# ssufujia/SPCBPT-OptiX7

Hardware: AMD Instinct MI355X
Metric: Mpaths/sec (whole node), SPCBPT, 1920x1080 (higher is better)
Workload: dtype f32; 1 GPU; bedroom scene read from glTF (986132 triangles, SAH BVH of 246804 quantised 4-wide nodes, depth 16), 1920x1080, SPCBPT: 100000 light paths + 2073600 eye paths per subframe, CONNECTION_N=3, subspace tuple: trained, light pass geometry 100000 cores x 1 paths x 52 slots (lane); warmup_steps_run=32, frames_in_flight=32, frames_per_eye_launch=32, light_passes_ahead=32, light_passes_per_launch=32, sampler_builds_ahead=32, parallelism=1 GPU, rccl_ranks=0

## Files before the change

### include/spcbpt.h

```cpp
#ifndef SPCBPT_H
#define SPCBPT_H

#include <stddef.h>
#include <stdint.h>

#ifdef __cplusplus
extern "C" {
#endif

#define SPCBPT_NUM_SUBSPACE 1000
#define SPCBPT_NUM_SUBSPACE_LIGHTSOURCE 200
#define SPCBPT_CONNECTION_N 3
#define SPCBPT_MIN_RR_RATE 0.3f
#define SPCBPT_SCENE_EPSILON 1e-3f

typedef enum spcbpt_status {
    SPCBPT_OK = 0,
    SPCBPT_ERR_INVALID_ARG = -1,
    SPCBPT_ERR_NO_DEVICE = -2,
    SPCBPT_ERR_HIP = -3,
    SPCBPT_ERR_UNKNOWN_ALG = -4,
    SPCBPT_ERR_STATE = -5,
    SPCBPT_ERR_CAPACITY = -6,
    SPCBPT_ERR_IO = -7
// ... 206 lines not shown
    int64_t pixels;
    double mean, max;
} spcbpt_film_error_stats;
int spcbpt_film_error_struct_size(void);
int spcbpt_film_error(spcbpt_ctx* ctx, spcbpt_film_error_stats* out);
int spcbpt_film_error_host(const float* accum_rgba, const float* m2n, int64_t n_pixels, spcbpt_film_error_stats* out);

#define SPCBPT_DENOISE_SIGMA_V 4.0f
int spcbpt_denoise_variance(spcbpt_ctx* ctx, const spcbpt_denoise_params* params);
int spcbpt_denoise_variance_host(const float* accum_rgba, const float* m2n, const float* albedo_rgba, const float* normal_depth_rgba,
                                 const float eye[3], const float U[3], const float V[3], const float W[3],
                                 int width, int height, const spcbpt_denoise_params* params, float* out_rgba);

typedef struct spcbpt_reproject_params {
    float sigma_n, sigma_x, max_history;
} spcbpt_reproject_params;
#define SPCBPT_REPROJECT_SIGMA_N 0.5f
#define SPCBPT_REPROJECT_SIGMA_X_FRACTION 0.002f
#define SPCBPT_REPROJECT_MAX_HISTORY 32.0f
int spcbpt_reproject_params_struct_size(void);
int spcbpt_history_capture(spcbpt_ctx* ctx, uint32_t frames);
int spcbpt_history_reproject(spcbpt_ctx* ctx, const spcbpt_reproject_params* params);
int spcbpt_history_resolve(spcbpt_ctx* ctx, uint32_t frames);
int spcbpt_history_reset(spcbpt_ctx* ctx);
int spcbpt_read_history(spcbpt_ctx* ctx, float* resolved_rgba, uint8_t* resolved_rgba8, float* prior_rgba, float* history_rgbn);
int spcbpt_history_reproject_host(const float eye[3], const float U[3], const float V[3], const float W[3], const float* normal_depth_rgba,
                                  const float eye_h[3], const float U_h[3], const float V_h[3], const float W_h[3],
                                  const float* history_normal_depth_rgba, const float* history_rgbn, int width, int height,
                                  const spcbpt_reproject_params* params, float sigma_x_default_diag, float* prior_out);
int spcbpt_history_resolve_host(const float* prior_rgba, const float* accum_rgba, uint32_t frames, int64_t n_pixels, float* out_rgba);

int spcbpt_history_denoise(spcbpt_ctx* ctx, const spcbpt_denoise_params* params);
int spcbpt_read_history_variance(spcbpt_ctx* ctx, float* resolved_var, float* prior_var, float* history_var);
int spcbpt_history_reproject_var_host(const float eye[3], const float U[3], const float V[3], const float W[3], const float* normal_depth_rgba,
                                      const float eye_h[3], const float U_h[3], const float V_h[3], const float W_h[3],
                                      const float* history_normal_depth_rgba, const float* history_rgbn, const float* history_var,
                                      int width, int height, const spcbpt_reproject_params* params, float sigma_x_default_diag,
                                      float* prior_out, float* prior_var_out);
int spcbpt_history_resolve_var_host(const float* prior_rgba, const float* prior_var, const float* accum_rgba, const float* m2n, uint32_t frames,
                                    int64_t n_pixels, float* out_rgba, float* out_var);
int spcbpt_history_denoise_host(const float* resolved_rgba, const float* resolved_var, const float* albedo_rgba, const float* normal_depth_rgba,
                                const float eye[3], const float U[3], const float V[3], const float W[3],
                                int width, int height, const spcbpt_denoise_params* params, float* out_rgba);

int spcbpt_get_counters(spcbpt_ctx* ctx, spcbpt_counters* out);
int spcbpt_reset_counters(spcbpt_ctx* ctx);
int spcbpt_debug_phase_clocks(spcbpt_ctx* ctx, uint64_t out[19]);
const char* spcbpt_build_source_hash(void);
const char* spcbpt_build_arithmetic(void);
int spcbpt_abi_struct_sizes(int32_t* sizes, int capacity);
int spcbpt_debug_spill_arm(spcbpt_ctx* ctx);
int spcbpt_debug_spill_count(spcbpt_ctx* ctx, uint64_t* words_written, int* entries_per_thread);

enum { SPCBPT_SAMPLER_SUBSPACE = 0, SPCBPT_SAMPLER_UNIFORM = 1 };
int spcbpt_set_connection_sampler(spcbpt_ctx* ctx, int mode);

typedef struct spcbpt_unit_eye_vertex {
    float position[3], normal[3], flux[3], color[3], last_position[3], rmis3[3];
    float pdf, single_pdf, last_normal_projection;
    int32_t material_id, subspace_id, depth, last_zone_id;
} spcbpt_unit_eye_vertex;
enum spcbpt_unit_op { SPCBPT_UNIT_BSDF = 0, SPCBPT_UNIT_TREE = 1, SPCBPT_UNIT_STAGE1 = 2, SPCBPT_UNIT_BSEARCH = 3, SPCBPT_UNIT_STAGE2 = 4,
                      SPCBPT_UNIT_UNIFORM = 5, SPCBPT_UNIT_CONNECT = 6, SPCBPT_UNIT_EYE_STEP = 7, SPCBPT_UNIT_SKY_MISS = 8,
                      SPCBPT_UNIT_STAGE2_GUIDED = 9, SPCBPT_UNIT_SORTED = 10, SPCBPT_UNIT_ENV = 11, SPCBPT_UNIT_ENV_TABLE = 12,
                      SPCBPT_UNIT_TEX = 13 };
int spcbpt_debug_unit(spcbpt_ctx* ctx, int op, const uint32_t* in, int in_words, uint32_t* out, int out_words, int n,
                      const float* aux, int aux_floats);

int spcbpt_debug_trace_bench(spcbpt_ctx* ctx, const float* rays, int n, int mode, int any, int repeat, float* out_t, int32_t* out_tri,
                             float* out_uv, int32_t* out_visible, double* avg_ms, uint64_t stats[5]);
int spcbpt_enable_counters(spcbpt_ctx* ctx, int enabled);

int spcbpt_stream(spcbpt_ctx* ctx, void** stream);
int spcbpt_sync(spcbpt_ctx* ctx);
int spcbpt_sync_light(spcbpt_ctx* ctx);
int spcbpt_launch_deferred(spcbpt_ctx* ctx, const char* alg, uint32_t subframe_index, int row_begin, int row_end, int row_step);
int spcbpt_merge_deferred(spcbpt_ctx* ctx, int keep);
int spcbpt_sync_film(spcbpt_ctx* ctx);
int spcbpt_launch_eye_batch(spcbpt_ctx* ctx, int n_frames, const uint32_t* subframes, int row_begin, int row_end, int row_step);
int spcbpt_launch_light_batch(spcbpt_ctx* ctx, uint32_t first_frame, int n_frames);
int spcbpt_build_sampler_batch(spcbpt_ctx* ctx, int n_builds);
int spcbpt_debug_batch_scratch(spcbpt_ctx* ctx, int64_t* bytes, int* frames, int* fallbacks);
int spcbpt_debug_read_sampling_tables(spcbpt_ctx* ctx, uint32_t* guide2, int capacity2, uint16_t* guide1, float* gamma_q);

int spcbpt_set_light_ahead(spcbpt_ctx* ctx, int on);
int spcbpt_get_pipeline_state(spcbpt_ctx* ctx, int* light_ahead, int* pending_passes, int* sampler_intact, int* deferred_outstanding);
int spcbpt_reuse_sampler(spcbpt_ctx* ctx);
int spcbpt_lvc_import_wait(spcbpt_ctx* ctx);

int spcbpt_kernel_time(spcbpt_ctx* ctx, const char* name, double* avg_ms, int* launches);
int spcbpt_reset_kernel_time(spcbpt_ctx* ctx);
int spcbpt_enable_kernel_timing(spcbpt_ctx* ctx, int enabled);

int spcbpt_trace_closest(spcbpt_ctx* ctx, const float* rays, int n,
                         float* out_t, int32_t* out_tri, float* out_uv);
int spcbpt_trace_any(spcbpt_ctx* ctx, const float* rays, int n, int32_t* out_visible);

typedef struct spcbpt_pretrace_path {
    float contri[3];
    float sample_pdf;
    float fix_pdf;
    int32_t begin_ind;
    int32_t end_ind;
    int32_t choice_id;
    int32_t pixel_id[2];
    int32_t valid;
    int32_t pad;
} spcbpt_pretrace_path;

typedef struct spcbpt_pretrace_node {
    float a_position[3];
    float b_position[3];
    float a_dir[3];
    float b_dir[3];
    float a_normal[3];
    float b_normal[3];
    float peak_pdf;
    int32_t path_id;
    int32_t label_a;
    int32_t label_b;
    int32_t valid;
    int32_t light_source;
} spcbpt_pretrace_node;

int spcbpt_set_pretrace(spcbpt_ctx* ctx, int num_core, int padding);

int spcbpt_train_records_count(spcbpt_ctx* ctx, int* n_paths, int* n_nodes);
int spcbpt_train_records_read(spcbpt_ctx* ctx, spcbpt_pretrace_path* paths, int cap_paths,
                              spcbpt_pretrace_node* nodes, int cap_nodes);
int spcbpt_train_records_import(spcbpt_ctx* ctx, const spcbpt_pretrace_path* paths, int n_paths,
                                const spcbpt_pretrace_node* nodes, int n_nodes);
int spcbpt_train_records_clear(spcbpt_ctx* ctx);

int spcbpt_preprocess(spcbpt_ctx* ctx, int target_paths, int target_q_paths, int train);
int spcbpt_preprocess_stage(spcbpt_ctx* ctx, int stage, int arg);
int spcbpt_get_gamma(spcbpt_ctx* ctx, float* gamma);

int spcbpt_checkpoint_write(const char* dir, const spcbpt_tree_node* eye_tree, int n_eye,
                            const spcbpt_tree_node* light_tree, int n_light, const float* q, const float* gamma);
int spcbpt_checkpoint_read(const char* dir, spcbpt_tree_node* eye_tree, int* n_eye, int cap_eye,
                           spcbpt_tree_node* light_tree, int* n_light, int cap_light, float* q, float* gamma,
                           int have_current_gamma);
int spcbpt_gamma_to_cmf(const float* gamma, float* cmf_gamma);
int spcbpt_checkpoint_save(spcbpt_ctx* ctx, const char* dir);
int spcbpt_checkpoint_load(spcbpt_ctx* ctx, const char* dir);

int spcbpt_image_load(const char* path, int* width, int* height, uint8_t* rgba, size_t capacity_bytes);

typedef struct spcbpt_viewer spcbpt_viewer;
typedef struct spcbpt_viewer_state {
    float eye[3], lookat[3], up[3];
    float U[3], V[3], W[3];
    float fov_y, aspect;
    int32_t width, height;
    uint32_t subframe_index;
    int32_t alg_id;
    int32_t should_close, one_frame_render_only, camera_changed;
    float render_fps;
} spcbpt_viewer_state;
int spcbpt_viewer_create(spcbpt_ctx* ctx, const float eye[3], const float lookat[3], const float up[3], float fov_y,
                         int width, int height, spcbpt_viewer** out);
void spcbpt_viewer_destroy(spcbpt_viewer* v);
int spcbpt_viewer_mouse_button(spcbpt_viewer* v, int button, int action, double x, double y);
int spcbpt_viewer_cursor_pos(spcbpt_viewer* v, double x, double y);
int spcbpt_viewer_scroll(spcbpt_viewer* v, double xscroll, double yscroll);
int spcbpt_viewer_window_size(spcbpt_viewer* v, int width, int height);
// ... 36 lines not shown
```

### spcbpt-optix7_amd/api.py

```python
from __future__ import annotations

import ctypes as C
import os
from dataclasses import dataclass, field
from typing import List, Optional

import numpy as np

NUM_SUBSPACE = 1000
NUM_SUBSPACE_LIGHTSOURCE = 200
CONNECTION_N = 3
ENV_EYE_SEES_SKY = 1
ENV_PT_SKY_SHADOW_ALONG_DIR = 2

_HERE = os.path.dirname(os.path.abspath(__file__))
LIB_PATH = os.path.join(_HERE, "csrc", "libspcbpt_hip.so")
FAST_LIB_PATH = os.path.join(_HERE, "csrc", "libspcbpt_hip_fast.so")


class Material(C.Structure):
    _fields_ = [("base_color", C.c_float * 3), ("metallic", C.c_float), ("roughness", C.c_float),
                ("specular", C.c_float), ("specular_tint", C.c_float), ("subsurface", C.c_float),
                ("sheen", C.c_float), ("sheen_tint", C.c_float), ("clearcoat", C.c_float),
                ("clearcoat_gloss", C.c_float), ("albedo_tex", C.c_int32), ("brdf", C.c_int32)]
# ... 597 lines not shown
    return et[:ne.value].copy(), lt[:nl.value].copy(), q, g.reshape(NUM_SUBSPACE, NUM_SUBSPACE)


def gamma_to_cmf(gamma):
    lib = load_library()
    g = np.ascontiguousarray(gamma, dtype=np.float32).reshape(-1)
    out = np.zeros_like(g)
    lib.spcbpt_gamma_to_cmf(g.ctypes.data, out.ctypes.data)
    return out.reshape(NUM_SUBSPACE, NUM_SUBSPACE)


def load_library(path: str = LIB_PATH):
    global _lib
    if _lib is not None:
        return _lib
    if os.environ.get("SPCBPT_LIB"):
        path = os.environ["SPCBPT_LIB"]
    if not os.path.exists(path):
        raise SpcbptError(f"{path} not built: run `python -c 'import __graft_entry__ as g; g.build()'` (no CPU fallback exists)")
    try:
        import torch
    except ImportError:
        pass
    lib = C.CDLL(path, mode=C.RTLD_GLOBAL)
    try:
        lib.spcbpt_build_source_hash.restype = C.c_char_p
        built = lib.spcbpt_build_source_hash().decode()
    except AttributeError:
        built = "none"
    if path in (LIB_PATH, FAST_LIB_PATH) and built != source_hash() and not os.environ.get("SPCBPT_ALLOW_STALE_LIB"):
        raise SpcbptError(f"{path} was built from other sources (library {built}, tree {source_hash()}): run `make -C spcbpt-optix7_amd/csrc`")
    vp, i32, u32, f32p = C.c_void_p, C.c_int, C.c_uint32, C.POINTER(C.c_float)
    sig = {
        "spcbpt_create": [C.POINTER(SceneDesc), i32, C.POINTER(vp)],
        "spcbpt_create_lit": [C.POINTER(SceneDesc), C.POINTER(MeshLight), i32, i32, C.POINTER(vp)],
        "spcbpt_mesh_light_struct_size": [],
        "spcbpt_light_info": [vp, i32, C.POINTER(i32), C.POINTER(C.c_float), C.POINTER(i32), C.POINTER(i32), C.POINTER(i32)],
        "spcbpt_mesh_light_table": [vp, i32, vp, i32, i32, vp, vp, vp, vp, C.POINTER(C.c_double), C.POINTER(i32)],
        "spcbpt_scene_file_mesh_lights": [vp, C.POINTER(C.POINTER(MeshLight)), C.POINTER(i32)],
        "spcbpt_destroy": [vp],
        "spcbpt_set_camera": [vp, f32p, f32p, f32p, f32p],
        "spcbpt_set_camera_lookat": [vp, f32p, f32p, f32p, C.c_float, C.c_float],
        "spcbpt_resize": [vp, i32, i32],
        "spcbpt_set_subspace": [vp, vp, i32, vp, i32, vp, vp],
        "spcbpt_set_light_trace": [vp, C.POINTER(LightTraceParams)],
        "spcbpt_launch": [vp, C.c_char_p, u32, i32, i32, i32],
        "spcbpt_build_sampler": [vp],
        "spcbpt_build_sampler_batch": [vp, C.c_int],
        "spcbpt_launch_eye_batch": [vp, i32, C.POINTER(u32), i32, i32, i32],
        "spcbpt_launch_light_batch": [vp, u32, i32],
        "spcbpt_lvc_export": [vp, C.POINTER(vp), C.POINTER(vp), C.POINTER(i32)],
        "spcbpt_lvc_import": [vp, vp, i32, i32],
        "spcbpt_set_environment": [vp, vp, i32, i32, vp, C.c_float],
        "spcbpt_get_environment": [vp, C.POINTER(i32), C.POINTER(i32), f32p, C.POINTER(C.c_float), C.POINTER(i32)],
        "spcbpt_set_environment_mode": [vp, i32],
        "spcbpt_get_environment_mode": [vp, C.POINTER(i32)],
        "spcbpt_hdr_load": [C.c_char_p, C.POINTER(i32), C.POINTER(i32), vp, C.c_size_t],
        "spcbpt_lvc_set_capacity": [vp, i32],
        "spcbpt_lvc_get_capacity": [vp, C.POINTER(i32), C.POINTER(i32)],
        "spcbpt_lvc_read": [vp, vp, i32, C.POINTER(i32)],
        "spcbpt_sampler_read": [vp, vp, vp, vp, i32, C.POINTER(i32), C.POINTER(i32)],
        "spcbpt_read_accum": [vp, vp],
        "spcbpt_read_frame": [vp, vp],
        "spcbpt_accum_device_ptr": [vp, C.POINTER(vp)],
        "spcbpt_clear_accum": [vp],
        "spcbpt_get_counters": [vp, C.POINTER(Counters)],
        "spcbpt_reset_counters": [vp],
        "spcbpt_debug_phase_clocks": [vp, C.POINTER(C.c_uint64)],
        "spcbpt_set_connection_sampler": [vp, i32],
        "spcbpt_debug_unit": [vp, i32, vp, i32, vp, i32, i32, vp, i32],
        "spcbpt_debug_trace_bench": [vp, vp, i32, i32, i32, i32, vp, vp, vp, vp, vp, vp],
        "spcbpt_debug_spill_arm": [vp],
        "spcbpt_debug_spill_count": [vp, C.POINTER(C.c_uint64), C.POINTER(i32)],
        "spcbpt_enable_counters": [vp, i32],
        "spcbpt_stream": [vp, C.POINTER(vp)],
        "spcbpt_sync": [vp], "spcbpt_sync_film": [vp], "spcbpt_merge_deferred": [vp, i32], "spcbpt_launch_deferred": [vp, C.c_char_p, u32, i32, i32, i32],
        "spcbpt_sync_light": [vp],
        "spcbpt_set_light_ahead": [vp, i32],
        "spcbpt_get_pipeline_state": [vp, C.POINTER(i32), C.POINTER(i32), C.POINTER(i32), C.POINTER(i32)],
        "spcbpt_reuse_sampler": [vp],
        "spcbpt_read_film": [vp, vp, vp],
        "spcbpt_debug_batch_scratch": [vp, C.POINTER(C.c_int64), C.POINTER(i32), C.POINTER(i32)],
        "spcbpt_debug_read_sampling_tables": [vp, vp, i32, vp, vp],
        "spcbpt_lvc_import_wait": [vp],
        "spcbpt_kernel_time": [vp, C.c_char_p, C.POINTER(C.c_double), C.POINTER(i32)],
        "spcbpt_reset_kernel_time": [vp],
        "spcbpt_enable_kernel_timing": [vp, i32],
        "spcbpt_trace_closest": [vp, vp, i32, vp, vp, vp],
        "spcbpt_trace_any": [vp, vp, i32, vp],
        "spcbpt_camera_splat": [f32p, f32p, f32p, f32p, i32, i32, f32p, f32p, f32p, C.POINTER(i32), C.POINTER(i32), f32p],
        "spcbpt_launch_features": [vp, u32, i32, i32, i32],
        "spcbpt_read_features": [vp, vp, vp],
        "spcbpt_denoise": [vp, C.POINTER(DenoiseParams)],
        "spcbpt_denoise_params_struct_size": [],
        "spcbpt_read_denoised": [vp, vp, vp],
        "spcbpt_denoise_host": [f32p, f32p, f32p, f32p, f32p, f32p, f32p, i32, i32, C.POINTER(DenoiseParams), f32p],
        "spcbpt_set_film_moments": [vp, i32],
        "spcbpt_get_film_moments": [vp, C.POINTER(i32)],
        "spcbpt_read_film_moments": [vp, vp],
        "spcbpt_film_moments_update_host": [f32p, f32p, u32, C.c_int64, f32p],
        "spcbpt_film_error": [vp, C.POINTER(FilmErrorStats)],
        "spcbpt_film_error_struct_size": [],
        "spcbpt_film_error_host": [f32p, f32p, C.c_int64, C.POINTER(FilmErrorStats)],
        "spcbpt_denoise_variance": [vp, C.POINTER(DenoiseParams)],
        "spcbpt_history_capture": [vp, C.c_uint32], "spcbpt_history_reproject": [vp, C.POINTER(ReprojectParams)], "spcbpt_history_resolve": [vp, C.c_uint32],
        "spcbpt_history_reset": [vp], "spcbpt_reproject_params_struct_size": [], "spcbpt_read_history": [vp, vp, vp, vp, vp],
        "spcbpt_history_reproject_host": [f32p, f32p, f32p, f32p, f32p, f32p, f32p, f32p, f32p, f32p, f32p, i32, i32, C.POINTER(ReprojectParams), C.c_float, f32p],
        "spcbpt_history_resolve_host": [f32p, f32p, C.c_uint32, C.c_int64, f32p],
        "spcbpt_history_denoise": [vp, C.POINTER(DenoiseParams)], "spcbpt_read_history_variance": [vp, vp, vp, vp],
        "spcbpt_history_reproject_var_host": [f32p, f32p, f32p, f32p, f32p, f32p, f32p, f32p, f32p, f32p, f32p, f32p, i32, i32, C.POINTER(ReprojectParams), C.c_float, f32p, f32p],
        "spcbpt_history_resolve_var_host": [f32p, f32p, f32p, f32p, C.c_uint32, C.c_int64, f32p, f32p],
        "spcbpt_history_denoise_host": [f32p, f32p, f32p, f32p, f32p, f32p, f32p, f32p, i32, i32, C.POINTER(DenoiseParams), f32p],
        "spcbpt_viewer_set_denoise": [vp, i32], "spcbpt_viewer_get_denoise": [vp, C.POINTER(i32)],
        "spcbpt_viewer_set_reproject": [vp, i32], "spcbpt_viewer_get_reproject": [vp, C.POINTER(i32), C.POINTER(i32)],
        "spcbpt_denoise_variance_host": [f32p, f32p, f32p, f32p, f32p, f32p, f32p, f32p, i32, i32, C.POINTER(DenoiseParams), f32p],
        "spcbpt_preprocess": [vp, i32, i32, i32],
        "spcbpt_set_pretrace": [vp, i32, i32],
        "spcbpt_train_records_count": [vp, C.POINTER(i32), C.POINTER(i32)],
        "spcbpt_train_records_read": [vp, vp, i32, vp, i32],
        "spcbpt_train_records_import": [vp, vp, i32, vp, i32],
        "spcbpt_train_records_clear": [vp],
        "spcbpt_preprocess_stage": [vp, i32, i32],
        "spcbpt_get_gamma": [vp, vp],
        "spcbpt_checkpoint_write": [C.c_char_p, vp, i32, vp, i32, vp, vp],
        "spcbpt_checkpoint_read": [C.c_char_p, vp, C.POINTER(i32), i32, vp, C.POINTER(i32), i32, vp, vp, i32],
        "spcbpt_gamma_to_cmf": [vp, vp],
        "spcbpt_viewer_create": [vp, f32p, f32p, f32p, C.c_float, i32, i32, C.POINTER(vp)],
        "spcbpt_viewer_mouse_button": [vp, i32, i32, C.c_double, C.c_double],
        "spcbpt_viewer_cursor_pos": [vp, C.c_double, C.c_double],
        "spcbpt_viewer_scroll": [vp, C.c_double, C.c_double],
        "spcbpt_viewer_window_size": [vp, i32, i32],
        "spcbpt_viewer_iconify": [vp, i32],
        "spcbpt_viewer_key": [vp, i32, i32],
        "spcbpt_viewer_set_fps": [vp, C.c_float],
        "spcbpt_viewer_set_light_ahead": [vp, i32], "spcbpt_viewer_set_pipeline": [vp, i32],
        "spcbpt_viewer_frame": [vp],
        "spcbpt_viewer_get_state": [vp, C.POINTER(ViewerState)],
        "spcbpt_image_load": [C.c_char_p, C.POINTER(i32), C.POINTER(i32), vp, C.c_size_t],
        "spcbpt_checkpoint_save": [vp, C.c_char_p],
        "spcbpt_checkpoint_load": [vp, C.c_char_p],
        "spcbpt_gltf_load": [C.c_char_p, C.POINTER(vp), C.c_char_p, i32],
        "spcbpt_scene_file_load": [C.c_char_p, C.c_char_p, C.POINTER(vp)],
        "spcbpt_scene_file_desc": [vp, C.POINTER(SceneDesc)],
        "spcbpt_scene_file_camera": [vp, f32p, f32p, f32p, f32p, C.POINTER(i32), C.POINTER(i32)],
        "spcbpt_scene_file_environment": [vp, C.POINTER(vp), C.POINTER(i32), C.POINTER(i32), f32p, C.POINTER(C.c_float)],
        "spcbpt_scene_file_free": [vp],
        "spcbpt_get_subspace": [vp, vp, C.POINTER(i32), i32, vp, C.POINTER(i32), i32, vp, vp],
        "spcbpt_scene_info": [vp, C.POINTER(i32), C.POINTER(i32), C.POINTER(i32)],
    }
    for name, args in sig.items():
        if os.environ.get("SPCBPT_LIB") and not hasattr(lib, name):
            continue
        fn = getattr(lib, name)
        fn.argtypes = args
        fn.restype = C.c_int
    lib.spcbpt_viewer_destroy.argtypes = [vp]
    lib.spcbpt_viewer_destroy.restype = None
    lib.spcbpt_viewer_alg_name.argtypes = [i32]
    lib.spcbpt_viewer_alg_name.restype = C.c_char_p
    lib.spcbpt_last_error.argtypes = [vp]
    lib.spcbpt_last_error.restype = C.c_char_p
    lib.spcbpt_build_arithmetic.restype = C.c_char_p
    lib.spcbpt_scene_file_warnings.argtypes = [vp]
    lib.spcbpt_scene_file_warnings.restype = C.c_char_p
    _lib = lib
    return lib


EXPORTED_SYMBOLS = [
    "spcbpt_create", "spcbpt_create_lit", "spcbpt_mesh_light_struct_size", "spcbpt_light_info", "spcbpt_mesh_light_table", "spcbpt_scene_file_mesh_lights", "spcbpt_destroy", "spcbpt_last_error", "spcbpt_set_camera", "spcbpt_set_camera_lookat",
    "spcbpt_resize", "spcbpt_set_subspace", "spcbpt_set_light_trace", "spcbpt_launch", "spcbpt_launch_eye_batch", "spcbpt_launch_light_batch", "spcbpt_build_sampler", "spcbpt_build_sampler_batch",
    "spcbpt_lvc_export", "spcbpt_lvc_import", "spcbpt_lvc_set_capacity", "spcbpt_lvc_get_capacity", "spcbpt_set_environment", "spcbpt_get_environment", "spcbpt_set_environment_mode", "spcbpt_get_environment_mode", "spcbpt_hdr_load", "spcbpt_lvc_read", "spcbpt_sampler_read", "spcbpt_read_accum",
    "spcbpt_read_frame", "spcbpt_accum_device_ptr", "spcbpt_clear_accum", "spcbpt_get_counters",
    "spcbpt_reset_counters", "spcbpt_debug_phase_clocks", "spcbpt_debug_spill_arm", "spcbpt_debug_spill_count", "spcbpt_set_connection_sampler", "spcbpt_debug_unit", "spcbpt_debug_trace_bench",
    "spcbpt_build_source_hash", "spcbpt_build_arithmetic", "spcbpt_abi_struct_sizes", "spcbpt_lvc_export_on", "spcbpt_lvc_import_gathered", "spcbpt_lvc_export_batch_on", "spcbpt_lvc_import_gathered_batch", "spcbpt_film_pack_bands", "spcbpt_film_unpack_bands", "spcbpt_image_size", "spcbpt_get_light_trace", "spcbpt_enable_counters", "spcbpt_stream", "spcbpt_sync", "spcbpt_sync_light", "spcbpt_launch_deferred", "spcbpt_merge_deferred", "spcbpt_sync_film", "spcbpt_set_light_ahead", "spcbpt_get_pipeline_state", "spcbpt_reuse_sampler", "spcbpt_read_film", "spcbpt_debug_batch_scratch", "spcbpt_debug_read_sampling_tables", "spcbpt_lvc_import_wait", "spcbpt_kernel_time",
    "spcbpt_reset_kernel_time", "spcbpt_enable_kernel_timing", "spcbpt_trace_closest", "spcbpt_trace_any", "spcbpt_camera_splat",
    "spcbpt_launch_features", "spcbpt_read_features", "spcbpt_denoise", "spcbpt_denoise_params_struct_size", "spcbpt_read_denoised", "spcbpt_denoise_host",
    "spcbpt_set_film_moments", "spcbpt_get_film_moments", "spcbpt_read_film_moments", "spcbpt_film_moments_update_host", "spcbpt_film_error", "spcbpt_film_error_struct_size", "spcbpt_film_error_host", "spcbpt_denoise_variance", "spcbpt_denoise_variance_host",
    "spcbpt_history_capture", "spcbpt_history_reproject", "spcbpt_history_resolve", "spcbpt_history_reset", "spcbpt_read_history", "spcbpt_reproject_params_struct_size",
    "spcbpt_history_reproject_host", "spcbpt_history_resolve_host", "spcbpt_viewer_set_reproject", "spcbpt_viewer_get_reproject",
    "spcbpt_history_denoise", "spcbpt_read_history_variance", "spcbpt_history_reproject_var_host", "spcbpt_history_resolve_var_host", "spcbpt_history_denoise_host",
    "spcbpt_viewer_set_denoise", "spcbpt_viewer_get_denoise",
    "spcbpt_preprocess", "spcbpt_get_subspace", "spcbpt_scene_info", "spcbpt_set_pretrace", "spcbpt_train_records_count",
    "spcbpt_train_records_read", "spcbpt_train_records_import", "spcbpt_train_records_clear", "spcbpt_preprocess_stage",
    "spcbpt_get_gamma", "spcbpt_gltf_load", "spcbpt_scene_file_load", "spcbpt_scene_file_desc", "spcbpt_scene_file_camera",
    "spcbpt_scene_file_warnings", "spcbpt_scene_file_environment", "spcbpt_scene_file_free",
    "spcbpt_viewer_create", "spcbpt_viewer_destroy", "spcbpt_viewer_mouse_button", "spcbpt_viewer_cursor_pos", "spcbpt_viewer_scroll",
    "spcbpt_viewer_window_size", "spcbpt_viewer_iconify", "spcbpt_viewer_key", "spcbpt_viewer_set_fps", "spcbpt_viewer_set_light_ahead", "spcbpt_viewer_set_pipeline", "spcbpt_viewer_frame",
    "spcbpt_viewer_get_state", "spcbpt_viewer_alg_name",
    "spcbpt_image_load", "spcbpt_checkpoint_write", "spcbpt_checkpoint_read", "spcbpt_gamma_to_cmf", "spcbpt_checkpoint_save", "spcbpt_checkpoint_load",
]


def _fp(a):
    return a.ctypes.data_as(C.POINTER(C.c_float))


class Renderer:

    def __init__(self, scene: Scene, device: int = 0):
        self.lib = load_library()
        self.scene = scene
        sd, keep = scene.desc()
        h = C.c_void_p()
        if scene.mesh_lights:
            ml = scene.mesh_light_array()
            rc = self.lib.spcbpt_create_lit(C.byref(sd), ml, len(scene.mesh_lights), device, C.byref(h))
        else:
            rc = self.lib.spcbpt_create(C.byref(sd), device, C.byref(h))
        if rc != 0:
            msg = self.lib.spcbpt_last_error(None)
            raise SpcbptError(f"spcbpt_create failed ({rc}): {msg.decode() if msg else ''}")
        self.h = h
        self.width = self.height = 0
        self.lt = None

    def _chk(self, rc, what):
        if rc != 0:
            msg = self.lib.spcbpt_last_error(self.h)
            raise SpcbptError(f"{what} failed ({rc}): {msg.decode() if msg else ''}")

    def close(self):
        if getattr(self, "h", None):
            self.lib.spcbpt_destroy(self.h)
            self.h = None

    def __del__(self):
        try:
            self.close()
        except Exception:
            pass

    def set_camera(self, eye, U, V, W):
        a = [np.ascontiguousarray(x, dtype=np.float32) for x in (eye, U, V, W)]
        self._chk(self.lib.spcbpt_set_camera(self.h, *[_fp(x) for x in a]), "set_camera")

    def set_camera_lookat(self, eye, lookat, up, fov, aspect):
        a = [np.ascontiguousarray(x, dtype=np.float32) for x in (eye, lookat, up)]
        self._chk(self.lib.spcbpt_set_camera_lookat(self.h, *[_fp(x) for x in a], fov, aspect), "set_camera_lookat")

    def resize(self, w, h):
        self._chk(self.lib.spcbpt_resize(self.h, w, h), "resize")
        self.width, self.height = w, h

    def set_subspace(self, eye_tree=None, light_tree=None, q=None, cmf_gamma=None):
        if eye_tree is None and light_tree is None and q is None and cmf_gamma is None:
            self._chk(self.lib.spcbpt_set_subspace(self.h, None, 0, None, 0, None, None), "set_subspace")
            return
        et = np.ascontiguousarray(eye_tree, dtype=TREE_NODE_DTYPE)
        lt = np.ascontiguousarray(light_tree, dtype=TREE_NODE_DTYPE)
        q = np.ascontiguousarray(q, dtype=np.float32)
        g = np.ascontiguousarray(cmf_gamma, dtype=np.float32)
        assert q.size == NUM_SUBSPACE and g.size == NUM_SUBSPACE * NUM_SUBSPACE
        self._chk(self.lib.spcbpt_set_subspace(self.h, et.ctypes.data, et.shape[0], lt.ctypes.data, lt.shape[0],
                                               q.ctypes.data, g.ctypes.data), "set_subspace")

    def get_subspace(self, cap=1 << 20):
        et = np.zeros(cap, dtype=TREE_NODE_DTYPE)
# ... 126 lines not shown
        return out

    def read_features(self):
        self.image_size()
        a = np.zeros((self.height, self.width, 4), dtype=np.float32)
        n = np.zeros((self.height, self.width, 4), dtype=np.float32)
        self._chk(self.lib.spcbpt_read_features(self.h, a.ctypes.data, n.ctypes.data), "read_features")
        return a, n

    def read_film_moments(self):
        self.image_size()
        out = np.zeros((self.height, self.width, 4), dtype=np.float32)
        self._chk(self.lib.spcbpt_read_film_moments(self.h, out.ctypes.data), "read_film_moments")
        return out

    def history_capture(self, frames):
        self._chk(self.lib.spcbpt_history_capture(self.h, int(frames)), "history_capture")

    def history_reproject(self, sigma_n=0.0, sigma_x=0.0, max_history=0.0):
        p = ReprojectParams(float(sigma_n), float(sigma_x), float(max_history))
        self._chk(self.lib.spcbpt_history_reproject(self.h, C.byref(p)), "history_reproject")

    def history_resolve(self, frames):
        self._chk(self.lib.spcbpt_history_resolve(self.h, int(frames)), "history_resolve")

    def history_denoise(self, iterations=5, sigma_v=0.0, sigma_n=0.0, sigma_x=0.0):
        p = DenoiseParams(int(iterations), float(sigma_v), float(sigma_n), float(sigma_x))
        self._chk(self.lib.spcbpt_history_denoise(self.h, C.byref(p)), "history_denoise")

    def read_history_variance(self, resolved=True, prior=False, history=False):
        w, h = self.image_size()
        want = {"resolved": resolved, "prior": prior, "history": history}
        out = {k: np.zeros((h, w, 4), dtype=np.float32) for k, on in want.items() if on}
        self._chk(self.lib.spcbpt_read_history_variance(self.h, *[out[k].ctypes.data if k in out else None for k in want]), "read_history_variance")
        return out

    def history_reset(self):
        self._chk(self.lib.spcbpt_history_reset(self.h), "history_reset")

    def read_history(self, resolved=True, frame=True, prior=False, history=False):
        self.image_size()
        want = {"resolved": (resolved, np.float32), "frame": (frame, np.uint8), "prior": (prior, np.float32), "history": (history, np.float32)}
        out = {k: np.zeros((self.height, self.width, 4), dtype=t) for k, (on, t) in want.items() if on}
        self._chk(self.lib.spcbpt_read_history(self.h, *[out[k].ctypes.data if k in out else None for k in want]), "read_history")
        return out

    def read_denoised(self):
        self.image_size()
        d = np.zeros((self.height, self.width, 4), dtype=np.float32)
        f = np.zeros((self.height, self.width, 4), dtype=np.uint8)
        self._chk(self.lib.spcbpt_read_denoised(self.h, d.ctypes.data, f.ctypes.data), "read_denoised")
        return d, f

    def clear_accum(self):
        self._chk(self.lib.spcbpt_clear_accum(self.h), "clear_accum")

    def read_film(self, accum=True, frame=True):
        self.image_size()
        a = np.zeros((self.height, self.width, 4), dtype=np.float32) if accum else None
        f = np.zeros((self.height, self.width, 4), dtype=np.uint8) if frame else None
        self._chk(self.lib.spcbpt_read_film(self.h, a.ctypes.data if accum else None, f.ctypes.data if frame else None), "read_film")
        return a, f

    def pipeline_state(self):
        v = [C.c_int32() for _ in range(4)]
        self._chk(self.lib.spcbpt_get_pipeline_state(self.h, *[C.byref(x) for x in v]), "get_pipeline_state")
        return dict(zip(("light_ahead", "pending_passes", "sampler_intact", "deferred"), (int(x.value) for x in v)))

    def reuse_sampler(self):
        self._chk(self.lib.spcbpt_reuse_sampler(self.h), "reuse_sampler")

    def batch_scratch(self):
        b, f, k = C.c_int64(), C.c_int32(), C.c_int32()
        self._chk(self.lib.spcbpt_debug_batch_scratch(self.h, C.byref(b), C.byref(f), C.byref(k)), "debug_batch_scratch")
        return {"bytes": int(b.value), "frames": int(f.value), "fallbacks": int(k.value)}

    def sampling_tables(self, vertex_count):
        g2 = np.zeros(max(vertex_count, 1), dtype=np.uint32)
        g1 = np.zeros((NUM_SUBSPACE, 1024), dtype=np.uint16)
        gq = np.zeros((NUM_SUBSPACE, NUM_SUBSPACE), dtype=np.float32)
        self._chk(self.lib.spcbpt_debug_read_sampling_tables(self.h, g2.ctypes.data if vertex_count > 0 else None, len(g2), g1.ctypes.data, gq.ctypes.data),
                  "debug_read_sampling_tables")
        return g2[:vertex_count], g1, gq

    def lvc_read(self, capacity=None):
        if capacity is None:
            capacity = self.lt.num_core * self.lt.core_padding if self.lt else 1 << 22
        out = np.zeros(capacity, dtype=LIGHT_VERTEX_DTYPE)
        n = C.c_int()
        self._chk(self.lib.spcbpt_lvc_read(self.h, out.ctypes.data, capacity, C.byref(n)), "lvc_read")
        return out[:n.value].copy()

    def lvc_import(self, verts: np.ndarray):
        v = np.ascontiguousarray(verts, dtype=LIGHT_VERTEX_DTYPE)
        self._chk(self.lib.spcbpt_lvc_import(self.h, v.ctypes.data, v.shape[0], 0), "lvc_import")

    def lvc_import_device(self, d_ptr: int, count: int):
        self._chk(self.lib.spcbpt_lvc_import(self.h, C.c_void_p(d_ptr), count, 1), "lvc_import")

    def set_environment(self, rgba, center=None, radius=0.0):
        a = np.ascontiguousarray(rgba, dtype=np.float32)
        assert a.ndim == 3 and a.shape[2] == 4
        c3 = None if center is None else np.ascontiguousarray(center, dtype=np.float32)
        self._chk(self.lib.spcbpt_set_environment(self.h, a.ctypes.data, a.shape[1], a.shape[0], None if c3 is None else c3.ctypes.data, float(radius)), "set_environment")

    def environment(self):
        w, h, n = C.c_int(), C.c_int(), C.c_int()
        c3 = np.zeros(3, np.float32)
        r = C.c_float()
        self._chk(self.lib.spcbpt_get_environment(self.h, C.byref(w), C.byref(h), _fp(c3), C.byref(r), C.byref(n)), "get_environment")
        f = C.c_int()
        self._chk(self.lib.spcbpt_get_environment_mode(self.h, C.byref(f)), "get_environment_mode")
        return dict(width=w.value, height=h.value, center=c3, radius=r.value, n_lights=n.value, flags=f.value)

    def set_environment_mode(self, flags: int):
        self._chk(self.lib.spcbpt_set_environment_mode(self.h, int(flags)), "set_environment_mode")

    def lvc_set_capacity(self, vertices: int):
        self._chk(self.lib.spcbpt_lvc_set_capacity(self.h, int(vertices)), "lvc_set_capacity")

    def lvc_capacity(self):
        v, n = C.c_int(), C.c_int()
        self._chk(self.lib.spcbpt_lvc_get_capacity(self.h, C.byref(v), C.byref(n)), "lvc_get_capacity")
        return v.value, n.value

    def lvc_export(self):
        dv, dc, cap = C.c_void_p(), C.c_void_p(), C.c_int()
        self._chk(self.lib.spcbpt_lvc_export(self.h, C.byref(dv), C.byref(dc), C.byref(cap)), "lvc_export")
        return dv.value, dc.value, cap.value

    def sampler_read(self, capacity=None):
        if capacity is None:
            capacity = self.lt.num_core * self.lt.core_padding if self.lt else 1 << 22
        sub = np.zeros(NUM_SUBSPACE, dtype=SUBSPACE_DTYPE)
        cmfs = np.zeros(capacity, dtype=np.float32)
        jump = np.zeros(capacity, dtype=np.int32)
        vc, pc = C.c_int(), C.c_int()
        self._chk(self.lib.spcbpt_sampler_read(self.h, sub.ctypes.data, cmfs.ctypes.data, jump.ctypes.data, capacity,
                                               C.byref(vc), C.byref(pc)), "sampler_read")
        return sub, cmfs[:vc.value].copy(), jump[:vc.value].copy(), vc.value, pc.value

    def accum_device_ptr(self):
        p = C.c_void_p()
        self._chk(self.lib.spcbpt_accum_device_ptr(self.h, C.byref(p)), "accum_device_ptr")
        return p.value

    def set_light_ahead(self, on: bool):
        self._chk(self.lib.spcbpt_set_light_ahead(self.h, int(on)), "set_light_ahead")

    def lvc_import_wait(self):
        self._chk(self.lib.spcbpt_lvc_import_wait(self.h), "lvc_import_wait")

    def sync_light(self):
        self._chk(self.lib.spcbpt_sync_light(self.h), "sync_light")

    def stream(self):
        p = C.c_void_p()
        self._chk(self.lib.spcbpt_stream(self.h, C.byref(p)), "stream")
        return p.value or 0

    def counters(self):
        c = Counters()
        self._chk(self.lib.spcbpt_get_counters(self.h, C.byref(c)), "get_counters")
        return c.as_dict()

    def phase_clocks(self):
# ... 99 lines not shown
```

### spcbpt-optix7_amd/csrc/capi.hip

```cpp
#include "capi_common.h"
#include "mesh_light.h"

using namespace spc;

static thread_local std::string g_create_error;

static int create_context(const spcbpt_scene_desc* sc, const spcbpt_mesh_light* ml, int n_ml, int device, spcbpt_ctx** out) {
    if (!sc || !out) { g_create_error = "null argument"; return SPCBPT_ERR_INVALID_ARG; }
    *out = nullptr;
    if (!ml) {
        if (!sc->vertices || !sc->indices || !sc->tri_material || sc->n_vertices < 3 || sc->n_triangles < 1 || sc->n_materials < 1 ||
            !sc->materials || sc->n_lights < 1 || !sc->lights) {
            g_create_error = "scene needs vertices, indices, tri_material, >=1 material and >=1 quad light";
            return SPCBPT_ERR_INVALID_ARG;
        }
    } else {
        if (!sc->vertices || !sc->indices || !sc->tri_material || sc->n_vertices < 3 || sc->n_triangles < 1 || sc->n_materials < 1 ||
            !sc->materials || sc->n_lights < 0 || (sc->n_lights > 0 && !sc->lights) || n_ml < 0 || sc->n_lights + n_ml < 1) {
            g_create_error = "scene needs vertices, indices, tri_material, >=1 material and >=1 light (quad or mesh)";
            return SPCBPT_ERR_INVALID_ARG;
        }
    }
    int ndev = 0;
    if (hipGetDeviceCount(&ndev) != hipSuccess || ndev <= 0) { g_create_error = "no HIP device available (the MI355X path has no CPU fallback)"; return SPCBPT_ERR_NO_DEVICE; }
// ... 94 lines not shown
    for (int i = 0; i < sc->n_lights; i++) {
        const spcbpt_quad_light& s = sc->lights[i];
        DLight L;
        memset(&L, 0, sizeof(L));
        float cr[3] = {s.u[1] * s.v[2] - s.u[2] * s.v[1], s.u[2] * s.v[0] - s.u[0] * s.v[2], s.u[0] * s.v[1] - s.u[1] * s.v[0]};
        float len = sqrtf(cr[0] * cr[0] + cr[1] * cr[1] + cr[2] * cr[2]);
        if (!(len > 0)) { g_create_error = "degenerate quad light"; delete c; return SPCBPT_ERR_INVALID_ARG; }
        float inv = 1.0f / len;
        for (int k = 0; k < 3; k++) {
            L.corner[k] = s.position[k]; L.u[k] = s.position[k] + s.u[k]; L.v[k] = s.position[k] + s.v[k];
            L.emission[k] = s.emission[k]; L.normal[k] = cr[k] * inv;
        }
        L.area = len; L.div_level = s.div_level; L.ss_base = ss_base; L.id = (int)lights.size();
        ss_base += s.div_level * s.div_level;
        lights.push_back(L);
        DMaterial d;
        memset(&d, 0, sizeof(d));
        d.base_color[0] = d.base_color[1] = d.base_color[2] = 1.0f; d.metallic = 1.0f; d.roughness = 1.0f; d.specular = 0.5f;
        d.sheen_tint = 0.5f; d.clearcoat_gloss = 1.0f; d.light_id = i;
        mats.push_back(d);
        uint32_t base = (uint32_t)(V.size() / 3);
        float p3[3] = {L.u[0] + L.v[0] - L.corner[0], L.u[1] + L.v[1] - L.corner[1], L.u[2] + L.v[2] - L.corner[2]};
        V.insert(V.end(), L.corner, L.corner + 3); V.insert(V.end(), L.u, L.u + 3); V.insert(V.end(), L.v, L.v + 3); V.insert(V.end(), p3, p3 + 3);
        const float quv[8] = {0, 0, 1, 0, 0, 1, 1, 1};
        UV.insert(UV.end(), quv, quv + 8);
        const uint32_t qi[6] = {base, base + 1, base + 3, base, base + 3, base + 2};
        I.insert(I.end(), qi, qi + 6);
        TM.push_back((int)mats.size() - 1); TM.push_back((int)mats.size() - 1);
        EM.push_back(1); EM.push_back(1);
        c->h_light_tris.push_back(2);
    }
    for (int j = 0; j < n_ml; j++) {
        const MeshLightTable& T = ml_tables[(size_t)j];
        const int n = (int)T.tri.size();
        DLight L;
        memset(&L, 0, sizeof(L));
        L.area = (float)T.area; L.div_level = T.n_patches; L.ss_base = ss_base; L.id = (int)lights.size(); L.type = 2;
        for (int k = 0; k < 3; k++) L.emission[k] = ml[j].emission[k];
        ss_base += T.n_patches;
        DMaterial d;
        memset(&d, 0, sizeof(d));
        d.base_color[0] = d.base_color[1] = d.base_color[2] = 1.0f; d.metallic = 1.0f; d.roughness = 1.0f; d.specular = 0.5f;
        d.sheen_tint = 0.5f; d.clearcoat_gloss = 1.0f; d.light_id = L.id;
        mats.push_back(d);
        const int padded = (n + 7) / 8 * 8 + 8, buckets = mesh_light_guide_buckets(n);
        std::vector<uint32_t> guide;
        build_mesh_light_guide(T.cmf, buckets, guide);
        const size_t rec_off = c->h_etable.size() / 4, cmf_off = rec_off + (size_t)MESH_LIGHT_REC_QUADS * n, guide_off = cmf_off + (size_t)padded / 4;
        c->h_etable.resize((guide_off + (size_t)buckets / 4) * 4, 0.0f);
        const int32_t words[6] = {(int32_t)rec_off, (int32_t)cmf_off, (int32_t)guide_off, n, buckets, padded};
        memcpy(L.corner, words, 12); memcpy(L.u, words + 3, 12);
        for (int i = 0; i < n; i++) {
            const int t = ml_tris[(size_t)j][(size_t)T.tri[(size_t)i]];
            const uint32_t base = (uint32_t)(V.size() / 3);
            float P[3][3];
            for (int v = 0; v < 3; v++) {
                memcpy(P[v], sc->vertices + 3 * (size_t)sc->indices[3 * (size_t)t + v], 12);
                V.insert(V.end(), P[v], P[v] + 3);
                UV.push_back((float)T.patch[(size_t)i] + 0.5f); UV.push_back(0.0f);
                I[3 * (size_t)t + v] = base + (uint32_t)v;
            }
            TM[(size_t)t] = (int)mats.size() - 1;
            EM[(size_t)t] = 1;
            float* r = &c->h_etable[(rec_off + (size_t)MESH_LIGHT_REC_QUADS * i) * 4];
            for (int k = 0; k < 3; k++) { r[k] = P[0][k]; r[4 + k] = P[1][k] - P[0][k]; r[8 + k] = P[2][k] - P[0][k]; }
            r[3] = T.cmf[(size_t)i];
            memcpy(r + 7, &T.patch[(size_t)i], 4);
        }
        float* cm = &c->h_etable[cmf_off * 4];
        for (int i = 0; i < padded; i++) cm[i] = i < n ? T.cmf[(size_t)i] : 2.0f;
        memcpy(&c->h_etable[guide_off * 4], guide.data(), (size_t)buckets * 4);
        lights.push_back(L);
        c->h_light_tris.push_back(n);
    }
    HostMesh mesh;
    mesh.vertices = V.data(); mesh.texcoords = UV.data(); mesh.indices = I.data(); mesh.tri_material = TM.data(); mesh.tri_emitter = EM.data();
    mesh.n_vertices = (int)(V.size() / 3); mesh.n_triangles = (int)(I.size() / 3);
    Lbvh bvh;
    build_lbvh(mesh, bvh);
    c->n_triangles = mesh.n_triangles; c->n_nodes = (int)(bvh.nodes.size() / 16); c->bvh_depth = bvh.depth;
    c->n_lights = (int)lights.size(); c->n_mats = (int)mats.size();

    CREATE_TRY(c->d_nodes.reserve(bvh.nodes.size() + bvh.pairs.size()));
    CREATE_TRY(c->d_tris.reserve(bvh.tris.size()));
    if (getenv("SPCBPT_NO_TRI_PAIRS")) {
        for (size_t i = 0; i < bvh.pairs.size() / 16; i++) { uint32_t fl; memcpy(&fl, &bvh.pairs[i * 16 + 15], 4); fl &= 0x80000000u; memcpy(&bvh.pairs[i * 16 + 15], &fl, 4); }
        bvh.n_paired = 0;
    }
    CREATE_TRY(hipMemcpy(c->d_nodes + bvh.nodes.size(), bvh.pairs.data(), bvh.pairs.size() * 4, hipMemcpyHostToDevice));
    c->n_paired = bvh.n_paired;
    CREATE_TRY(c->d_tri_orig.reserve(bvh.tri_orig.size()));
    CREATE_TRY(c->d_mats.reserve(mats.size()));
    CREATE_TRY(hipMemcpy(c->d_nodes, bvh.nodes.data(), bvh.nodes.size() * 4, hipMemcpyHostToDevice));
    CREATE_TRY(hipMemcpy(c->d_tris, bvh.tris.data(), bvh.tris.size() * 4, hipMemcpyHostToDevice));
    CREATE_TRY(hipMemcpy(c->d_tri_orig, bvh.tri_orig.data(), bvh.tri_orig.size() * 4, hipMemcpyHostToDevice));
    CREATE_TRY(hipMemcpy(c->d_mats, mats.data(), mats.size() * sizeof(DMaterial), hipMemcpyHostToDevice));
    c->h_lights = lights;
    for (int k = 0; k < 3; k++) { c->bbox_lo[k] = 1e30f; c->bbox_hi[k] = -1e30f; }
    for (size_t i = 0; i < V.size(); i += 3)
        for (int k = 0; k < 3; k++) { c->bbox_lo[k] = std::min(c->bbox_lo[k], V[i + k]); c->bbox_hi[k] = std::max(c->bbox_hi[k], V[i + k]); }
    std::vector<DTexture> texs;
    for (int i = 0; i < sc->n_textures; i++) {
        const spcbpt_texture& t = sc->textures[i];
        if (!t.rgba || t.width < 1 || t.height < 1) { g_create_error = "bad texture"; delete c; return SPCBPT_ERR_INVALID_ARG; }
        uint32_t* d = nullptr;
        CREATE_TRY(dev_alloc(&d, (size_t)t.width * t.height));
        c->d_tex_data.push_back(d);
        CREATE_TRY(hipMemcpy(d, t.rgba, (size_t)t.width * t.height * 4, hipMemcpyHostToDevice));
        texs.push_back(DTexture{d, t.width, t.height});
    }
    CREATE_TRY(c->d_tex.reserve(texs.size()));
    if (!texs.empty()) CREATE_TRY(hipMemcpy(c->d_tex, texs.data(), texs.size() * sizeof(DTexture), hipMemcpyHostToDevice));
    CREATE_TRY(c->d_set_counts_all.reserve((size_t)2 * Context::kMaxSets + 2));
    CREATE_TRY(hipMemset(c->d_set_counts_all, 0, (2 * Context::kMaxSets + 2) * sizeof(int)));
    for (int s = 0; s < c->n_sets; s++) {
        CREATE_TRY(c->sets[s].subspace.reserve((size_t)SPCBPT_NUM_SUBSPACE));
        c->sets[s].counts = c->d_set_counts_all + 2 * s;
    }
    {
        hipDeviceProp_t prop;
        CREATE_TRY(hipGetDeviceProperties(&prop, device));
        c->num_cus = prop.multiProcessorCount;
    }
    CREATE_TRY(c->d_work_counter.reserve((size_t)Context::kMaxRender + 2));
    for (int lane = 0; lane < 2; lane++) c->lanes[lane].work_counter = c->d_work_counter + Context::kMaxRender + lane;
    CREATE_TRY(c->d_diag.reserve((size_t)4));
    CREATE_TRY(hipMemset(c->d_diag, 0, 4 * sizeof(uint32_t)));
    if (const char* e = getenv("SPCBPT_DEBUG_SPILL_ENTRIES")) c->spill_entries_debug = std::max(0, atoi(e));
    CREATE_TRY(c->d_counters.reserve((size_t)C_COUNT));
    CREATE_TRY(hipMemset(c->d_counters, 0, C_COUNT * sizeof(unsigned long long)));
    memset(&c->kp, 0, sizeof(c->kp));
    if (c->upload_lights()) { g_create_error = c->error; delete c; return SPCBPT_ERR_HIP; }
    c->kp.scene.nodes = c->d_nodes; c->kp.scene.tris = c->d_tris; c->kp.scene.tri_base = c->n_nodes; c->kp.scene.tri_orig = c->d_tri_orig; c->kp.scene.mats = c->d_mats;
    c->kp.scene.lights = c->d_lights; c->kp.scene.tex = c->d_tex; c->kp.scene.n_lights = c->n_lights; c->kp.scene.n_mats = c->n_mats;
    CREATE_TRY(c->d_nodes_q.reserve((size_t)c->n_nodes * 16));
    launch_repack_nodes_quad(c->d_nodes, c->d_nodes_q, c->n_nodes, c->stream);
    CREATE_TRY(hipGetLastError());
    CREATE_TRY(hipStreamSynchronize(c->stream));
    c->kp.scene.nodes_q = getenv("SPCBPT_NO_QUAD_TAIL") ? nullptr : c->d_nodes_q.p;
    c->kp.scene.fan_tail = getenv("SPCBPT_NO_FAN_TAIL") ? 0 : 1;
    c->kp.scene.general = 0;
    for (const DMaterial& m : mats) if (m.brdf) c->kp.scene.general = 1;
    if (n_ml > 0) c->kp.scene.general = 1;
    c->kp.sampler_counts = c->sets[0].counts;
    c->kp.diag = c->d_diag;
    c->kp.row_step = 1;
    CREATE_TRY(hipDeviceSynchronize());
#undef CREATE_TRY
    *out = c;
    return SPCBPT_OK;
}

extern "C" {

int spcbpt_create(const spcbpt_scene_desc* sc, int device, spcbpt_ctx** out) { return create_context(sc, nullptr, 0, device, out); }

int spcbpt_create_lit(const spcbpt_scene_desc* sc, const spcbpt_mesh_light* mesh_lights, int n_mesh_lights, int device, spcbpt_ctx** out) {
    if (n_mesh_lights < 0 || (n_mesh_lights > 0 && !mesh_lights)) { g_create_error = "create_lit: null mesh-light array"; if (out) *out = nullptr; return SPCBPT_ERR_INVALID_ARG; }
    static const spcbpt_mesh_light none = {0, {0, 0, 0}, 1};
    return create_context(sc, n_mesh_lights > 0 ? mesh_lights : &none, n_mesh_lights, device, out);
}
int spcbpt_mesh_light_struct_size(void) { return (int)sizeof(spcbpt_mesh_light); }

int spcbpt_light_info(spcbpt_ctx* c, int light, int32_t* type, float* area, int32_t* n_triangles, int32_t* first_subspace, int32_t* n_patches) {
    CTX_CHECK(c);
    if (light < 0 || light >= (int)c->h_lights.size()) { c->error = "light_info: light index out of range (" + std::to_string(c->h_lights.size()) + " lights)"; return SPCBPT_ERR_INVALID_ARG; }
    const DLight& L = c->h_lights[(size_t)light];
    const DEnv& E = c->kp.scene.env;
    if (type) *type = L.type;
    if (area) *area = L.type == 1 ? 0.0f : L.area;
    if (n_triangles) *n_triangles = light < (int)c->h_light_tris.size() ? c->h_light_tris[(size_t)light] : 0;
    if (first_subspace) *first_subspace = SPCBPT_NUM_SUBSPACE - 1 - (L.type == 1 ? 0 : L.ss_base);
    if (n_patches) *n_patches = L.type == 1 ? E.div_level * E.div_level : (L.type == 2 ? L.div_level : L.div_level * L.div_level);
    return SPCBPT_OK;
}

int spcbpt_destroy(spcbpt_ctx* c) {
    if (!c) return SPCBPT_ERR_INVALID_ARG;
    spc_viewers_forget_context(c);
    (void)hipSetDevice(c->device);
    (void)c->sync_all();
    delete c;
    return SPCBPT_OK;
}

const char* spcbpt_build_arithmetic(void) {
#if defined(SPCBPT_FAST_MATH_BUILD)
    return "approx";
#else
    return "ieee";
#endif
}

const char* spcbpt_last_error(const spcbpt_ctx* c) { return c ? c->error.c_str() : g_create_error.c_str(); }


int spcbpt_set_camera(spcbpt_ctx* c, const float eye[3], const float U[3], const float V[3], const float W[3]) {
    CTX_CHECK(c);
    if (!eye || !U || !V || !W) { c->error = "null camera vector"; return SPCBPT_ERR_INVALID_ARG; }
    memcpy(c->kp.eye, eye, 12); memcpy(c->kp.U, U, 12); memcpy(c->kp.V, V, 12); memcpy(c->kp.W, W, 12);
    c->have_camera = true;
    return SPCBPT_OK;
}

int spcbpt_set_camera_lookat(spcbpt_ctx* c, const float eye[3], const float lookat[3], const float up[3], float fov, float aspect) {
    CTX_CHECK(c);
    if (!eye || !lookat || !up) { c->error = "null camera vector"; return SPCBPT_ERR_INVALID_ARG; }
    auto cross = [](const float* a, const float* b, float* r) { r[0] = a[1] * b[2] - a[2] * b[1]; r[1] = a[2] * b[0] - a[0] * b[2]; r[2] = a[0] * b[1] - a[1] * b[0]; };
    auto norm = [](float* v) { float inv = 1.0f / sqrtf(v[0] * v[0] + v[1] * v[1] + v[2] * v[2]); v[0] *= inv; v[1] *= inv; v[2] *= inv; };
    float W[3] = {lookat[0] - eye[0], lookat[1] - eye[1], lookat[2] - eye[2]}, U[3], V[3];
    float wlen = sqrtf(W[0] * W[0] + W[1] * W[1] + W[2] * W[2]);
    cross(W, up, U); norm(U);
    cross(U, W, V); norm(V);
    float vlen = wlen * tanf(0.5f * fov * 3.14159265358979323846f / 180.0f);
    for (int k = 0; k < 3; k++) V[k] *= vlen;
    float ulen = vlen * aspect;
// ... 134 lines not shown
```

### spcbpt-optix7_amd/csrc/capi_debug.hip

```cpp
#include "capi_common.h"

using namespace spc;

extern "C" {

int spcbpt_get_light_trace(spcbpt_ctx* c, spcbpt_light_trace_params* out) {
    CTX_CHECK(c);
    if (!out) return SPCBPT_ERR_INVALID_ARG;
    *out = c->lt;
    if (out->core_count == 0) out->core_count = out->num_core - out->core_begin;
    return SPCBPT_OK;
}
int spcbpt_image_size(spcbpt_ctx* c, int* w, int* h) { CTX_CHECK(c); if (w) *w = (int)c->kp.width; if (h) *h = (int)c->kp.height; return SPCBPT_OK; }

int spcbpt_lvc_read(spcbpt_ctx* c, spcbpt_light_vertex* out, int capacity, int* count) {
    CTX_CHECK(c);
    if (!count) return SPCBPT_ERR_INVALID_ARG;
    if (!c->sets[c->lset].lvc) { c->error = "no LVC"; return SPCBPT_ERR_STATE; }
    int rc = c->fetch_counts();
    if (rc) return rc;
    *count = c->lvc_count;
    if (!out) return SPCBPT_OK;
    if (capacity < c->lvc_count) { c->error = "lvc_read: buffer too small"; return SPCBPT_ERR_CAPACITY; }
    HIP_TRY(c, hipMemcpy(out, c->sets[c->lset].lvc, (size_t)c->lvc_count * sizeof(LightVertex), hipMemcpyDeviceToHost));
    return SPCBPT_OK;
}

int spcbpt_sampler_read(spcbpt_ctx* c, spcbpt_subspace* sub, float* cmfs, int32_t* jump, int capacity, int* vc, int* pc) {
    CTX_CHECK(c);
    if (!c->have_sampler) { c->error = "no sampler built"; return SPCBPT_ERR_STATE; }
    if (!sub || !vc || !pc) return SPCBPT_ERR_INVALID_ARG;
    if (c->sync_all()) return SPCBPT_ERR_HIP;
    std::vector<DSubspace> h(SPCBPT_NUM_SUBSPACE);
    const CacheSet& S = c->sets[c->eset];
    HIP_TRY(c, hipMemcpy(h.data(), S.subspace, h.size() * sizeof(DSubspace), hipMemcpyDeviceToHost));
    for (int i = 0; i < SPCBPT_NUM_SUBSPACE; i++) {
        sub[i].jump_bias = h[i].jump_bias; sub[i].id = i; sub[i].size = h[i].size; sub[i].sum_pmf = h[i].sum_pmf; sub[i].q = 0;
    }
    int hc[2] = {0, 0};
    HIP_TRY(c, hipMemcpy(hc, S.counts, sizeof(hc), hipMemcpyDeviceToHost));
    *vc = hc[0]; *pc = hc[1];
    if (cmfs && jump) {
        if (capacity < hc[0]) { c->error = "sampler_read: buffer too small"; return SPCBPT_ERR_CAPACITY; }
        HIP_TRY(c, hipMemcpy(cmfs, S.cmfs, (size_t)hc[0] * 4, hipMemcpyDeviceToHost));
        HIP_TRY(c, hipMemcpy(jump, S.jump, (size_t)hc[0] * 4, hipMemcpyDeviceToHost));
    }
    return SPCBPT_OK;
}

int spcbpt_read_accum(spcbpt_ctx* c, float* out) {
    CTX_CHECK(c);
    if (!out || !c->d_accum) { c->error = "no accum buffer"; return SPCBPT_ERR_STATE; }
    if (c->sync_all()) return SPCBPT_ERR_HIP;
    if (int rc = c->check_diag()) return rc;
    HIP_TRY(c, hipMemcpy(out, c->d_accum, (size_t)c->kp.width * c->kp.height * 16, hipMemcpyDeviceToHost));
    return SPCBPT_OK;
}
int spcbpt_read_frame(spcbpt_ctx* c, uint8_t* out) {
    CTX_CHECK(c);
    if (!out || !c->d_frame) { c->error = "no frame buffer"; return SPCBPT_ERR_STATE; }
    if (c->sync_all()) return SPCBPT_ERR_HIP;
    if (int rc = c->check_diag()) return rc;
    HIP_TRY(c, hipMemcpy(out, c->d_frame, (size_t)c->kp.width * c->kp.height * 4, hipMemcpyDeviceToHost));
    return SPCBPT_OK;
}
int spcbpt_read_film(spcbpt_ctx* c, float* accum_out, uint8_t* frame_out) {
    CTX_CHECK(c);
    if (!c->d_accum || !c->d_frame) { c->error = "no film (spcbpt_resize first)"; return SPCBPT_ERR_STATE; }
    if (!c->cstream) HIP_TRY(c, hipStreamCreateWithFlags(&c->cstream, hipStreamNonBlocking));
    if (c->last_merge_k >= 0) HIP_TRY(c, c->ev_merge[c->last_merge_k].wait_on(c->cstream));
    const size_t px = (size_t)c->kp.width * c->kp.height;
    if (accum_out) HIP_TRY(c, hipMemcpyAsync(accum_out, c->d_accum, px * 16, hipMemcpyDeviceToHost, c->cstream));
    if (frame_out) HIP_TRY(c, hipMemcpyAsync(frame_out, c->d_frame, px * 4, hipMemcpyDeviceToHost, c->cstream));
    HIP_TRY(c, hipStreamSynchronize(c->cstream));
    return c->check_diag();
}
int spcbpt_debug_batch_scratch(spcbpt_ctx* c, int64_t* bytes, int* frames, int* fallbacks) {
    CTX_CHECK(c);
    if (bytes) *bytes = c->sbb_keys ? (int64_t)((size_t)c->sbb_frames * c->sbb_capacity * 16 + (size_t)c->sbb_frames * sampler_build_hist_ints() * sizeof(int)) : 0;
    if (frames) *frames = c->sbb_frames;
    if (fallbacks) *fallbacks = c->sbb_fallbacks;
    return SPCBPT_OK;
}
int spcbpt_debug_read_sampling_tables(spcbpt_ctx* c, uint32_t* guide2, int capacity2, uint16_t* guide1, float* gamma_q) {
    CTX_CHECK(c);
    if (c->sync_all()) return SPCBPT_ERR_HIP;
    if (guide2) {
        if (!c->have_sampler) { c->error = "no sampler built"; return SPCBPT_ERR_STATE; }
        int hc[2] = {0, 0};
        HIP_TRY(c, hipMemcpy(hc, c->sets[c->eset].counts, sizeof(hc), hipMemcpyDeviceToHost));
        if (capacity2 < hc[0]) { c->error = "debug_read_sampling_tables: buffer too small"; return SPCBPT_ERR_CAPACITY; }
        HIP_TRY(c, hipMemcpy(guide2, c->sets[c->eset].guide, (size_t)hc[0] * 4, hipMemcpyDeviceToHost));
    }
    if ((guide1 || gamma_q) && !c->d_guide1) { c->error = "no subspace tuple installed"; return SPCBPT_ERR_STATE; }
    if (guide1) HIP_TRY(c, hipMemcpy(guide1, c->d_guide1, (size_t)SPCBPT_NUM_SUBSPACE * CMF_GUIDE1 * sizeof(uint16_t), hipMemcpyDeviceToHost));
    if (gamma_q) HIP_TRY(c, hipMemcpy(gamma_q, c->d_gamma_q, (size_t)SPCBPT_NUM_SUBSPACE * SPCBPT_NUM_SUBSPACE * sizeof(float), hipMemcpyDeviceToHost));
    return SPCBPT_OK;
}
int spcbpt_accum_device_ptr(spcbpt_ctx* c, void** p) {
    CTX_CHECK(c);
    if (!p || !c->d_accum) return SPCBPT_ERR_STATE;
    *p = c->d_accum;
    return SPCBPT_OK;
}
int spcbpt_clear_accum(spcbpt_ctx* c) {
    CTX_CHECK(c);
    if (!c->d_accum) return SPCBPT_ERR_STATE;
    if (c->deferred.active) { c->error = "clear_accum: a deferred frame is outstanding (its merge would land in the cleared film): spcbpt_merge_deferred(ctx, keep) first"; return SPCBPT_ERR_STATE; }
    if (c->sync_all()) return SPCBPT_ERR_HIP;
    HIP_TRY(c, hipMemsetAsync(c->d_accum, 0, (size_t)c->kp.width * c->kp.height * 16, c->rstreams[0]));
    if (c->d_m2n) HIP_TRY(c, hipMemsetAsync(c->d_m2n, 0, (size_t)c->kp.width * c->kp.height * 16, c->rstreams[0]));
    HIP_TRY(c, hipStreamSynchronize(c->rstreams[0]));
    return SPCBPT_OK;
}

int spcbpt_get_counters(spcbpt_ctx* c, spcbpt_counters* o) {
    CTX_CHECK(c);
    if (!o) return SPCBPT_ERR_INVALID_ARG;
    unsigned long long h[C_COUNT];
    if (c->sync_all()) return SPCBPT_ERR_HIP;
    HIP_TRY(c, hipMemcpy(h, c->d_counters, sizeof(h), hipMemcpyDeviceToHost));
    o->closest_rays = h[C_CLOSEST]; o->shadow_rays = h[C_SHADOW]; o->node_visits = h[C_NODE]; o->tri_tests = h[C_TRI];
    o->surface_vertices = h[C_VERTEX]; o->textured_hits = h[C_TEX]; o->tree_nodes = h[C_TREE]; o->cmf_probes = h[C_CMF];
    o->connections = h[C_CONN]; o->gamma_q_reads = h[C_GQ]; o->lvc_stores = h[C_LVCW]; o->pixel_samples = h[C_PIX];
    o->eye_paths = h[C_EYE]; o->light_paths = h[C_LIGHT];
    return SPCBPT_OK;
}
int spcbpt_debug_phase_clocks(spcbpt_ctx* c, uint64_t out[19]) {
    CTX_CHECK(c);
    if (!out) return SPCBPT_ERR_INVALID_ARG;
    unsigned long long h[C_COUNT];
    if (c->sync_all()) return SPCBPT_ERR_HIP;
    HIP_TRY(c, hipMemcpy(h, c->d_counters, sizeof(h), hipMemcpyDeviceToHost));
    for (int i = 0; i < 5; i++) out[i] = h[C_PUBLIC + i] << 4;
    for (int i = 5; i < 9; i++) out[i] = h[C_PUBLIC + i];
    out[9] = h[C_T_SAMPLE] << 4;
    out[10] = h[C_W_START_MIN]; out[11] = h[C_W_END_MAX]; out[12] = h[C_W_END_SUM]; out[13] = h[C_W_WAVES]; out[14] = h[C_U_TAIL_SLOTS]; out[15] = h[C_U_TAIL_CLOSEST]; out[16] = h[C_U_TAIL_SHADOW]; out[17] = h[C_U_JOB_SLOTS]; out[18] = h[C_U_JOB_LANES];
    return SPCBPT_OK;
}
int spcbpt_reset_counters(spcbpt_ctx* c) {
    CTX_CHECK(c);
    if (c->sync_all()) return SPCBPT_ERR_HIP;
    HIP_TRY(c, hipMemsetAsync(c->d_counters, 0, C_COUNT * sizeof(unsigned long long), c->stream));
    HIP_TRY(c, hipMemsetAsync(c->d_counters + C_W_START_MIN, 0xff, sizeof(unsigned long long), c->stream));
    return SPCBPT_OK;
}
int spcbpt_enable_counters(spcbpt_ctx* c, int on) { CTX_CHECK(c); c->counting = on != 0; c->count_executed = on == 2; return SPCBPT_OK; }

int spcbpt_stream(spcbpt_ctx* c, void** s) { CTX_CHECK(c); if (!s) return SPCBPT_ERR_INVALID_ARG; *s = (void*)c->stream; return SPCBPT_OK; }
int spcbpt_set_light_ahead(spcbpt_ctx* c, int on) {
    CTX_CHECK(c);
    if (c->deferred.active) { c->error = "set_light_ahead: a deferred frame is outstanding: spcbpt_merge_deferred(ctx, keep) first"; return SPCBPT_ERR_STATE; }
    if (c->sync_all()) return SPCBPT_ERR_HIP;
    const bool was = c->light_ahead;
    c->light_ahead = on != 0;
    c->pending.clear();
    if (was && !c->light_ahead) { c->free_batch_build_scratch(); c->sbb_refused_bytes = 0; }
    return SPCBPT_OK;
}

int spcbpt_get_pipeline_state(spcbpt_ctx* c, int* light_ahead, int* pending_passes, int* sampler_intact, int* deferred_outstanding) {
    CTX_CHECK(c);
    if (light_ahead) *light_ahead = c->light_ahead ? 1 : 0;
    if (pending_passes) *pending_passes = (int)c->pending.size();
    if (sampler_intact) *sampler_intact = c->sampler_intact() ? 1 : 0;
    if (deferred_outstanding) *deferred_outstanding = c->deferred.active ? 1 : 0;
    return SPCBPT_OK;
}

int spcbpt_reuse_sampler(spcbpt_ctx* c) {
    CTX_CHECK(c);
    if (!c->sampler_intact()) { c->error = "reuse_sampler: the tables of the last sampler build are gone (a light pass, an import or a new tuple took their set)"; return SPCBPT_ERR_STATE; }
    c->have_sampler = true;
    return SPCBPT_OK;
}

int spcbpt_lvc_import_wait(spcbpt_ctx* c) {
    CTX_CHECK(c);
    if (c->import_gen >= 2 && c->ev_import[c->import_gen & 1]) HIP_TRY(c, hipEventSynchronize(c->ev_import[c->import_gen & 1]));
// ... 236 lines not shown
```

### spcbpt-optix7_amd/csrc/context.h

```cpp
#pragma once
#include <hip/hip_runtime.h>

#include <deque>
#include <map>
#include <string>
#include <type_traits>
#include <utility>
#include <vector>

#include "layout.h"
#include "reproject_pixel.h"

namespace spc {

struct Preprocessor;

struct TimedSpan {
    std::string name;
    hipEvent_t a, b;
    hipStream_t s;
};

template <class T>
static hipError_t dev_alloc(T** p, size_t n) {
// ... 42 lines not shown
struct CacheSet {
    DevBuf<LightVertex> lvc;
    DevBuf<LightVertex> lvc_sorted;
    DevBuf<uint32_t> jump;
    DevBuf<float> cmfs;
    DevBuf<uint32_t> guide;
    DevBuf<DSubspace> subspace;
    int* counts = nullptr;
    Event light;
    Event sampler, render;
    int render_event_of = 0;
    Event on_stream;
    int bound = -1;
    Event exch;
    int count_host = -1;
    bool light_counts_valid = false;
    int light_lane = 0;
};

struct LightLane {
    hipStream_t stream = nullptr;
    DevBuf<LightVertex> scratch;
    DevBuf<int> core_counts, core_offsets;
    DevBuf<uint32_t> keys, vals;
    DevBuf<float> weights;
    DevBuf<unsigned char> temp;
    DevBuf<uint32_t> spill;
    uint32_t* work_counter = nullptr;
};

struct Context {
    int device = 0;
    hipStream_t stream = nullptr;
    hipStream_t rstream = nullptr;
    hipStream_t cstream = nullptr;
    static const int kMaxRender = 8, kMaxSets = 128;
    int n_render = 2, n_sets = 6;
    hipStream_t rstreams[kMaxRender] = {};
    int rk = 0, last_merge_k = -1;
    DevBuf<float> d_result[kMaxRender];
    Event ev_merge[kMaxRender];
    CacheSet sets[kMaxSets];
    int lset = 0, eset = 0;
    std::deque<int> pending;
    bool light_ahead = false;
    int keys_set = -1;
    int export_on(hipStream_t xs, void** dv, void** dc, int* cap);
    int import_gathered(const void* shards, const int* counts_all, int world, int shard_cap, hipStream_t xs, int nf);
    int export_batch_on(hipStream_t xs, int nf, void* send, int* send_counts, int shard_cap);
    int wait_for_contents(hipStream_t xs, int s);
    hipEvent_t ev_import[2] = {};
    long long import_gen = 0;
    int* h_import_counts = nullptr;
    int* h_light_counts = nullptr;
    int build_set() const { return pending.empty() ? lset : pending.front(); }
    int begin_rewrite(hipStream_t ls, int s, int& waited_for);
    void set_rewritten(int s);
    int pass_traced(hipStream_t ls, int s, int lane);
    int sampler_built(int s);
    void contents_imported(int s, int count_host, int bound);
    template <class P>
    void sampler_tables(P& d, int s) const {
        const CacheSet& S = sets[s];
        d.lvc = S.lvc; d.lvc_sorted = S.lvc_sorted; d.subspace = S.subspace; d.cmfs = S.cmfs; d.guide = S.guide; d.sampler_counts = S.counts;
        if constexpr (std::is_same<P, KParams>::value) d.jump = reinterpret_cast<const int32_t*>(S.jump.p);
    }
    LightLane lanes[2];
    int light_toggle = 0;
    int ensure_lane_b();
    int light_pass_params(uint32_t frame, int n_frames, LightVertex* scratch, int* core_counts, bool count_events, DevBuf<uint32_t>& spill, int grid_cap);
    DevBuf<LightVertex> lb_scratch;
    DevBuf<int> lb_core_counts, lb_core_offsets, lb_path_counts;
    DevBuf<uint32_t> lb_spill;
    int launch_light_batch(uint32_t first_frame, int n);
    DevBuf<int> d_set_counts_all;
    DevBuf<uint32_t> d_spill_rs[kMaxRender];
    int sync_all();
    std::string error;
    KParams kp;
    DevBuf<float> d_nodes;
    DevBuf<float> d_nodes_q;
    DevBuf<float> d_nodes_q2;
    DevBuf<float> d_tris;
    int n_paired = 0;
    DevBuf<int32_t> d_tri_orig;
    DevBuf<DMaterial> d_mats;
    DLight* d_lights = nullptr;
    DevBuf<DTexture> d_tex;
    std::vector<uint32_t*> d_tex_data;
    int n_triangles = 0, n_nodes = 0, bvh_depth = 0, n_lights = 0, n_mats = 0;
    float* d_env_tex = nullptr;
    float* d_env_cmf = nullptr;
    std::vector<DLight> h_lights;
    std::vector<float> h_etable;
    std::vector<int> h_light_tris;
    int upload_lights();
    float bbox_lo[3] = {0, 0, 0}, bbox_hi[3] = {0, 0, 0};
    int set_environment(const float* rgba, int w, int h, const float* center, float radius);
    DevBuf<float> d_accum;
    DevBuf<uint32_t> d_frame;
    bool have_camera = false;
    float* d_eye_tree = nullptr;
    float* d_light_tree = nullptr;
    DevBuf<float> d_Q;
    DevBuf<float> d_gamma;
    DevBuf<float> d_gamma2;
    DevBuf<float> d_gamma_q;
    DevBuf<uint16_t> d_guide1;
    bool gamma_monotone = false;
    std::vector<spcbpt_tree_node> h_eye_tree, h_light_tree;
    std::vector<float> h_Q, h_gamma;
    bool have_subspace = false;
    bool tree_has_direction = false;
    spcbpt_light_trace_params lt = {100000, 52, 1, 0, 100000, 1};
    size_t lvc_capacity = 0;
    size_t lvc_fixed = 0;
    bool lvc_probe_needed = false;
    int probe_lvc_capacity();
    DevBuf<uint32_t> d_keys2;
    DevBuf<double> d_wsorted, d_prefix;
    DevBuf<int> d_hist;
    bool counting_build = true;
    int lvc_count = 0, path_count = 0;
    bool keys_ready = false, have_sampler = false;
    DevBuf<uint32_t> d_diag;
    int spill_entries_debug = -1;
    int spill_entries_needed() const;
    int check_diag();
    DevBuf<uint32_t> d_work_counter;
    int num_cus = 0, blocks_per_cu[3] = {0, 0, 0};
    int blocks_per_cu_batch = 0;
    int grid_percent = 0;
    int light_blocks_wide = -1;
    int light_blocks = -1;
    int light_batch_blocks = -1;
    int tiles_per_wave = 1;
    DevBuf<unsigned long long> d_counters;
    bool counting = false, timing = false;
    bool count_executed = false;
    int kernel_variant() const { return tree_has_direction ? 1 : (counting ? (count_executed ? 2 : 1) : 0); }
    std::vector<TimedSpan> spans;
    std::map<std::string, std::pair<double, int>> times;

    ~Context();
    void time_begin(const char* name, hipStream_t s = nullptr);
    void time_end();
    void resolve_spans();
    int ensure_spill(size_t threads, bool render = false);
    int ensure_temp(size_t bytes);
    int ensure_lvc_capacity(size_t n);
    int upload_tree(const spcbpt_tree_node* t, int n, float*& d_tree, std::vector<spcbpt_tree_node>& host_copy);
    int install_subspace(const spcbpt_tree_node* et, int ne, const spcbpt_tree_node* lt, int nl, const float* q, const float* g);
    int install_minimal_tuple();
    int set_light_trace(const spcbpt_light_trace_params& p);
    int launch_light(uint32_t frame);
    int fetch_counts();
    int fetch_counts_of(int set);
    int build_sampler();
    int build_sampler_batch(int n);
    DevBuf<uint32_t> sbb_keys; DevBuf<float> sbb_weights; DevBuf<double> sbb_wsorted; DevBuf<int> sbb_hist;
    int sbb_frames = 0; size_t sbb_capacity = 0;
    int sbb_fallbacks = 0;
    size_t sbb_refused_bytes = 0;
    void free_batch_build_scratch();
    size_t sbb_debug_limit() const;
    bool sampler_intact() const { return !built_sets.empty() && built_sets.back() == eset && sets[eset].sampler.set; }
    int launch_render(const char* name, bool spcbpt_alg, uint32_t frame, int r0, int r1, int rs, bool full_mis = false, bool defer_merge = false);
    struct Deferred { bool active = false; int rk = 0; uint32_t subframe = 0; int row_begin = 0, row_end = 0, row_step = 1; float* result = nullptr; } deferred;
    int merge_deferred(bool keep);
    int sync_film();
    std::deque<int> built_sets;
    int eye_batch = 1;
    DevBuf<float> d_result_b[kMaxRender][kMaxBatchFrames];
    DevBuf<FrameDesc> d_frames[kMaxRender];
    static const int kDescRing = 4;
    FrameDesc* h_frames = nullptr;
    hipEvent_t ev_desc[kMaxRender][kDescRing] = {};
    int desc_gen[kMaxRender] = {};
    int launch_eye_batch(int n, const uint32_t* subframes, int r0, int r1, int rs);
    DevBuf<float> d_splat[kMaxRender];
    int launch_splat(uint32_t frame, int r0, int r1, int rs);
    int film_ready();
    int begin_render(int r0, int r1, int rs);
    void next_render_stream();
    int chain_wait();
    int chain_end();
    int render_done(int s);
    int finish_frame();
    DevBuf<float> d_feat_albedo, d_feat_normal_depth;
    DevBuf<float> d_dn_position, d_dn_ping, d_dn_pong, d_denoised;
    DevBuf<uint32_t> d_denoised_frame;
    bool have_features = false, have_denoised = false;
    int launch_features(uint32_t subframe, int r0, int r1, int rs);
    int denoise(const spcbpt_denoise_params& p);
    void free_features();
    bool film_moments = false;
    DevBuf<float> d_m2n;
    DevBuf<unsigned char> d_err_scratch;
    int set_film_moments(bool on);
    int moments_step();
    int film_error(spcbpt_film_error_stats* out);
    int denoise_variance(const spcbpt_denoise_params& p);
    void free_moments();
    DevBuf<float> d_hist_rgbn, d_hist_normal_depth, d_prior, d_resolved;
    DevBuf<uint32_t> d_resolved_frame;
    ReprojectCamera hist_camera = {};
    uint32_t hist_width = 0, hist_height = 0;
    bool have_history = false, prior_live = false, have_resolved = false;
    int history_ready(const char* what, bool need_features);
    int resolve_into(uint32_t frames, float* out, uint32_t* frame, float* out_var = nullptr);
    int history_capture(uint32_t frames);
    int history_reproject(const spcbpt_reproject_params& p);
    int history_resolve(uint32_t frames);
    void free_history();
    DevBuf<float> d_hist_var, d_prior_var, d_resolved_var;
    bool have_hist_var = false, have_prior_var = false, have_resolved_var = false;
    bool history_variance_now() const;
    int history_denoise(const spcbpt_denoise_params& p);
    Preprocessor* pre = nullptr;
    spcbpt_pretrace_path* d_pre_paths = nullptr;
    spcbpt_pretrace_node* d_pre_nodes = nullptr;
    size_t pre_capacity = 0;
    int pre_num_core = 100000, pre_padding = 10, pre_last_added = 0;
    int set_pretrace(int num_core, int padding);
    int launch_pretrace(uint32_t iteration);
    int preprocess_stage(int stage, int arg);
    int preprocess(int target_paths, int target_q_paths, bool train);
    void free_preprocess();
};

}
```

### spcbpt-optix7_amd/csrc/ctx_state.hip

```cpp
#include "capi_common.h"

using namespace spc;

namespace spc {

void Context::time_begin(const char* name, hipStream_t s) {
    if (!timing) return;
    TimedSpan sp;
    sp.name = name;
    sp.s = s ? s : stream;
    (void)hipEventCreate(&sp.a);
    (void)hipEventCreate(&sp.b);
    (void)hipEventRecord(sp.a, sp.s);
    spans.push_back(sp);
}
void Context::time_end() {
    if (!timing || spans.empty()) return;
    (void)hipEventRecord(spans.back().b, spans.back().s);
}
int Context::sync_all() {
    HIP_TRY(this, hipStreamSynchronize(stream));
    if (lanes[1].stream) HIP_TRY(this, hipStreamSynchronize(lanes[1].stream));
    for (int k = 0; k < n_render; k++)
        if (rstreams[k] && rstreams[k] != stream) HIP_TRY(this, hipStreamSynchronize(rstreams[k]));
    return 0;
}
void Context::resolve_spans() {
    for (auto& sp : spans) {
        (void)hipEventSynchronize(sp.b);
        float ms = 0.f;
        if (hipEventElapsedTime(&ms, sp.a, sp.b) == hipSuccess) {
            auto& acc = times[sp.name];
            acc.first += ms;
            acc.second += 1;
        }
        (void)hipEventDestroy(sp.a);
        (void)hipEventDestroy(sp.b);
    }
    spans.clear();
}

int Context::spill_entries_needed() const {
    const int entries = std::max(0, 3 * bvh_depth - kStackLds);
    return spill_entries_debug >= 0 ? std::min(entries, spill_entries_debug) : entries;
}
int Context::check_diag() {
    if (!d_diag) return 0;
    uint32_t h[4] = {0, 0, 0, 0};
    HIP_TRY(this, hipMemcpy(h, d_diag, sizeof(h), hipMemcpyDeviceToHost));
    if (h[0] == 0 && h[1] == 0 && h[2] == 0) return 0;
    HIP_TRY(this, hipMemsetAsync(d_diag, 0, sizeof(h), stream));
    HIP_TRY(this, hipStreamSynchronize(stream));
    if (h[0] == 0 && h[1] == 0) {
        error = "light-vertex cache overflow: a light pass produced more vertices than a buffer set holds (" + std::to_string(lvc_capacity) +
                ", sized from a probe pass); frames since the last sync are invalid -- fix the capacity with spcbpt_lvc_set_capacity";
        return SPCBPT_ERR_CAPACITY;
    }
    if (h[0] == 0) {
        error = "LVC exchange: a rank's shard did not fit the agreed shard capacity (or the gathered cache did not fit the LVC); frames since the last sync are invalid -- raise the capacity (spcbpt_comm_set_shard_capacity)";
        return SPCBPT_ERR_CAPACITY;
    }
    error = "traversal stack overflow: " + std::to_string(h[0]) + " entries did not fit LDS + spill area (BVH depth " + std::to_string(bvh_depth) +
            ", spill entries per thread " + std::to_string(spill_entries_needed()) + "); results since the last sync are invalid";
    return SPCBPT_ERR_STATE;
}

int Context::ensure_spill(size_t threads, bool render) {
    const int entries = spill_entries_needed();
    kp.spill_entries = entries;
    if (entries == 0) { kp.spill = nullptr; return 0; }
    DevBuf<uint32_t>& buf = render ? d_spill_rs[rk] : lanes[0].spill;
    HIP_TRY(this, buf.reserve(threads * (size_t)entries));
    kp.spill = buf;
    return 0;
}

int Context::upload_tree(const spcbpt_tree_node* t, int n, float*& d_tree, std::vector<spcbpt_tree_node>& host_copy) {
    for (int i = 0; i < n; i++) {
        if (t[i].leaf) {
            if (t[i].label < 0 || t[i].label >= SPCBPT_NUM_SUBSPACE) { error = "tree label out of range"; return SPCBPT_ERR_INVALID_ARG; }
        } else {
            if (t[i].type < 0 || t[i].type > 2) { error = "tree node type out of range"; return SPCBPT_ERR_INVALID_ARG; }
            for (int k = 0; k < 8; k++)
                if (t[i].child[k] < 0 || t[i].child[k] >= n) { error = "tree child index out of range"; return SPCBPT_ERR_INVALID_ARG; }
        }
    }
    host_copy.assign(t, t + n);
    const size_t budget = (size_t)16 * n + 64;
    std::vector<float> packed(4);
    std::vector<int> src(1, 0);
    for (size_t slot = 0; slot < src.size(); slot++) {
        const spcbpt_tree_node& nd = t[src[slot]];
        uint32_t meta;
        if (nd.leaf) {
            meta = TREE_LEAF_BIT | (uint32_t)nd.label;
        } else {
            const size_t base = src.size();
            if (base + 8 > budget || base + 8 >= (1u << 29)) { error = "tree is not a finite tree (shared or cyclic children)"; return SPCBPT_ERR_INVALID_ARG; }
            meta = ((uint32_t)nd.type << 29) | (uint32_t)base;
            for (int k = 0; k < 8; k++) src.push_back(nd.child[k]);
            packed.resize(src.size() * 4);
        }
        float* q = &packed[slot * 4];
        q[0] = nd.mid[0]; q[1] = nd.mid[1]; q[2] = nd.mid[2];
        memcpy(q + 3, &meta, 4);
    }
    dev_free(d_tree);
    HIP_TRY(this, dev_alloc(&d_tree, packed.size()));
    HIP_TRY(this, hipMemcpyAsync(d_tree, packed.data(), packed.size() * sizeof(float), hipMemcpyHostToDevice, stream));
    HIP_TRY(this, hipStreamSynchronize(stream));
    return 0;
}

int Context::install_subspace(const spcbpt_tree_node* et, int ne, const spcbpt_tree_node* lt, int nl, const float* q, const float* g) {
    if (!et || !lt || !q || !g || ne < 1 || nl < 1) { error = "set_subspace: all four of eye_tree, light_tree, q, cmf_gamma are required"; return SPCBPT_ERR_INVALID_ARG; }
    if (sync_all()) return SPCBPT_ERR_HIP;
    int rc = upload_tree(et, ne, d_eye_tree, h_eye_tree);
    if (rc) return rc;
    rc = upload_tree(lt, nl, d_light_tree, h_light_tree);
    if (rc) return rc;
    tree_has_direction = false;
    for (int i = 0; i < ne; i++) if (!et[i].leaf && et[i].type == 2) tree_has_direction = true;
    for (int i = 0; i < nl; i++) if (!lt[i].leaf && lt[i].type == 2) tree_has_direction = true;
    h_Q.assign(q, q + SPCBPT_NUM_SUBSPACE);
    h_gamma.assign(g, g + (size_t)SPCBPT_NUM_SUBSPACE * SPCBPT_NUM_SUBSPACE);
    HIP_TRY(this, d_Q.reserve(SPCBPT_NUM_SUBSPACE));
    HIP_TRY(this, d_gamma.reserve((size_t)SPCBPT_NUM_SUBSPACE * SPCBPT_NUM_SUBSPACE));
    HIP_TRY(this, hipMemcpyAsync(d_Q, h_Q.data(), h_Q.size() * 4, hipMemcpyHostToDevice, stream));
    HIP_TRY(this, hipMemcpyAsync(d_gamma, h_gamma.data(), h_gamma.size() * 4, hipMemcpyHostToDevice, stream));
    {
        std::vector<float> two((size_t)SPCBPT_NUM_SUBSPACE * CMF2_ROW, 2.0f);
        for (int e = 0; e < SPCBPT_NUM_SUBSPACE; e++) {
            float* row = &two[(size_t)e * CMF2_ROW];
            float* fine = row + CMF2_COARSE + CMF2_MID;
            memcpy(fine, &h_gamma[(size_t)e * SPCBPT_NUM_SUBSPACE], SPCBPT_NUM_SUBSPACE * sizeof(float));
            for (int m = 0; m < CMF2_MID; m++) row[CMF2_COARSE + m] = fine[8 * m + 7];
            for (int k = 0; k < CMF2_COARSE; k++) row[k] = fine[64 * k + 63];
        }
        HIP_TRY(this, d_gamma2.reserve(two.size()));
        HIP_TRY(this, hipMemcpy(d_gamma2, two.data(), two.size() * sizeof(float), hipMemcpyHostToDevice));
        {
            std::vector<float> gq((size_t)SPCBPT_NUM_SUBSPACE * SPCBPT_NUM_SUBSPACE);
            for (int e = 0; e < SPCBPT_NUM_SUBSPACE; e++) {
                const float* row = &h_gamma[(size_t)e * SPCBPT_NUM_SUBSPACE];
                for (int l = 0; l < SPCBPT_NUM_SUBSPACE; l++) {
                    const float g = l == 0 ? row[0] : row[l] - row[l - 1];
                    gq[(size_t)e * SPCBPT_NUM_SUBSPACE + l] = g / h_Q[l];
                }
            }
            HIP_TRY(this, d_gamma_q.reserve(gq.size()));
            HIP_TRY(this, hipMemcpy(d_gamma_q, gq.data(), gq.size() * sizeof(float), hipMemcpyHostToDevice));
        }
        {
            std::vector<uint16_t> guide((size_t)SPCBPT_NUM_SUBSPACE * CMF_GUIDE1);
            for (int e = 0; e < SPCBPT_NUM_SUBSPACE; e++) {
                const float* row = &h_gamma[(size_t)e * SPCBPT_NUM_SUBSPACE];
                int k = 0;
                for (int b = 0; b < CMF_GUIDE1; b++) {
                    const float t = (float)b / (float)CMF_GUIDE1;
                    while (k < SPCBPT_NUM_SUBSPACE && !(row[k] > t)) k++;
                    guide[(size_t)e * CMF_GUIDE1 + b] = (uint16_t)k;
                }
            }
            HIP_TRY(this, d_guide1.reserve(guide.size()));
            HIP_TRY(this, hipMemcpy(d_guide1, guide.data(), guide.size() * sizeof(uint16_t), hipMemcpyHostToDevice));
        }
        gamma_monotone = true;
        for (int e = 0; e < SPCBPT_NUM_SUBSPACE && gamma_monotone; e++) {
            const float* row = &h_gamma[(size_t)e * SPCBPT_NUM_SUBSPACE];
            for (int l = 1; l < SPCBPT_NUM_SUBSPACE; l++) if (!(row[l] >= row[l - 1])) { gamma_monotone = false; break; }
            if (!(row[SPCBPT_NUM_SUBSPACE - 1] >= 1.0f)) gamma_monotone = false;
        }
    }
    HIP_TRY(this, hipStreamSynchronize(stream));
    kp.eye_tree = d_eye_tree; kp.light_tree = d_light_tree; kp.Q = d_Q; kp.cmf_gamma = d_gamma; kp.cmf_gamma2 = gamma_monotone ? d_gamma2 : nullptr; kp.cmf_guide1 = d_guide1; kp.gamma_q = d_gamma_q;
    have_subspace = true;
    return 0;
}

int Context::upload_lights() {
    static_assert(sizeof(DLight) % 16 == 0, "the emitter-triangle table must start on a 16-B boundary");
    std::vector<unsigned char> blob(h_lights.size() * sizeof(DLight) + h_etable.size() * sizeof(float));
    memcpy(blob.data(), h_lights.data(), h_lights.size() * sizeof(DLight));
    if (!h_etable.empty()) memcpy(blob.data() + h_lights.size() * sizeof(DLight), h_etable.data(), h_etable.size() * sizeof(float));
    dev_free(d_lights);
    unsigned char* d = nullptr;
    HIP_TRY(this, dev_alloc(&d, blob.size()));
    d_lights = reinterpret_cast<DLight*>(d);
    HIP_TRY(this, hipMemcpy(d_lights, blob.data(), blob.size(), hipMemcpyHostToDevice));
    n_lights = (int)h_lights.size();
    kp.scene.lights = d_lights; kp.scene.n_lights = n_lights;
    return 0;
}

int Context::set_environment(const float* rgba, int w, int h, const float* center, float radius) {
    if (!rgba || w < 1 || h < 1 || (long long)w * h > (1ll << 26)) { error = "set_environment: bad image"; return SPCBPT_ERR_INVALID_ARG; }
    if (kp.scene.env.valid) { error = "set_environment: the context already has an environment map"; return SPCBPT_ERR_STATE; }
    int patches = 0;
    for (const DLight& L : h_lights) patches += L.type == 2 ? L.div_level : L.div_level * L.div_level;
    if (patches > SPCBPT_NUM_SUBSPACE_LIGHTSOURCE / 2) { error = "set_environment: with an environment map the quad lights may use at most 100 patch subspaces (sum of div_level^2)"; return SPCBPT_ERR_INVALID_ARG; }
    for (size_t i = 0; i < (size_t)w * h * 4; i++) if (!std::isfinite(rgba[i])) { error = "set_environment: non-finite texel"; return SPCBPT_ERR_INVALID_ARG; }
    if (sync_all()) return SPCBPT_ERR_HIP;
    std::vector<float> tex, cmf;
    env_build(rgba, w, h, tex, cmf);
    if (!(cmf.back() > 0.0f) || !std::isfinite(cmf.back())) { error = "set_environment: the image holds no energy"; return SPCBPT_ERR_INVALID_ARG; }
    const long long flat = env_first_undrawable(cmf);
// ... 200 lines not shown
```

### spcbpt-optix7_amd/csrc/dev_bsdf.h

```cpp
#pragma once
#include "device_lib.h"

namespace spc {

struct Pbr {
    f3 base;
    float metallic, roughness, specular, specularTint, subsurface, sheen, sheenTint, clearcoat, clearcoatGloss;
    int albedo_tex, light_id;
    int brdf;
};
SPC_DEV Pbr load_pbr(const DeviceScene& S, int id) {
    const float4* p = reinterpret_cast<const float4*>(S.mats + id);
    const float4 a = p[0], b = p[1], c = p[2], d = p[3];
    Pbr m;
    m.base = mk3(a.x, a.y, a.z); m.metallic = a.w;
    m.roughness = b.x; m.specular = b.y; m.specularTint = b.z; m.subsurface = b.w;
    m.sheen = c.x; m.sheenTint = c.y; m.clearcoat = c.z; m.clearcoatGloss = c.w;
    m.albedo_tex = __float_as_int(d.x); m.light_id = __float_as_int(d.y); m.brdf = __float_as_int(d.z);
    return m;
}
SPC_DEV Pbr load_pbr_colored(const DeviceScene& S, int id, f3 color) {
    Pbr m = load_pbr(S, id);
    m.base = color;
    return m;
}
SPC_DEV f3 tex_fetch_rgb(const DTexture& T, float u, float v) {
    const float x = u * (float)T.width - 0.5f, y = v * (float)T.height - 0.5f;
    const float fx = floorf(x), fy = floorf(y);
    const float ax = x - fx, ay = y - fy;
    int x0 = (int)fx % T.width, y0 = (int)fy % T.height;
    if (x0 < 0) x0 += T.width;
    if (y0 < 0) y0 += T.height;
    int x1 = x0 + 1 == T.width ? 0 : x0 + 1, y1 = y0 + 1 == T.height ? 0 : y0 + 1;
    const uint32_t t00 = T.rgba[(size_t)y0 * T.width + x0], t10 = T.rgba[(size_t)y0 * T.width + x1];
    const uint32_t t01 = T.rgba[(size_t)y1 * T.width + x0], t11 = T.rgba[(size_t)y1 * T.width + x1];
    const float w00 = (1 - ax) * (1 - ay), w10 = ax * (1 - ay), w01 = (1 - ax) * ay, w11 = ax * ay;
    const float s = 1.0f / 255.0f;
    f3 r;
    r.x = w00 * ((t00 & 255u) * s) + w10 * ((t10 & 255u) * s) + w01 * ((t01 & 255u) * s) + w11 * ((t11 & 255u) * s);
    r.y = w00 * (((t00 >> 8) & 255u) * s) + w10 * (((t10 >> 8) & 255u) * s) + w01 * (((t01 >> 8) & 255u) * s) + w11 * (((t11 >> 8) & 255u) * s);
    r.z = w00 * (((t00 >> 16) & 255u) * s) + w10 * (((t10 >> 16) & 255u) * s) + w01 * (((t01 >> 16) & 255u) * s) + w11 * (((t11 >> 16) & 255u) * s);
    return r;
}
struct Geom { f3 P, N; float u, v; int mat; bool emitter; };
SPC_DEV Geom local_geometry(const DeviceScene& S, const HitRec& h) {
    const size_t base = (size_t)h.tri * 4;
    const float4 a = ldq(S.tris, base), b = ldq(S.tris, base + 1), c = ldq(S.tris, base + 2), d = ldq(S.tris, base + 3);
    const f3 P0 = mk3(a.x, a.y, a.z), P1 = mk3(b.x, b.y, b.z), P2 = mk3(c.x, c.y, c.z);
    Geom g;
    const float w = 1.0f - h.u - h.v;
    g.P = w * P0 + h.u * P1 + h.v * P2;
    g.N = normalize(cross(P1 - P0, P2 - P0));
    g.u = w * a.w + h.u * c.w + h.v * d.y;
    g.v = w * b.w + h.u * d.x + h.v * d.z;
    const uint32_t meta = __float_as_uint(d.w);
    g.mat = (int)(meta & 0x7fffffffu);
    g.emitter = (meta & 0x80000000u) != 0;
    return g;
}
template <bool COUNT>
SPC_DEV void color_tex_sample(const DeviceScene& S, const Geom& g, Pbr& m, Counts<COUNT>& cn) {
    if (m.albedo_tex > 0) {
        const f3 t = tex_fetch_rgb(S.tex[m.albedo_tex - 1], g.u, g.v);
        m.base = mk3(powf(t.x, 2.2f), powf(t.y, 2.2f), powf(t.z, 2.2f));
        cn.add(C_TEX);
    }
}

struct Onb {
    f3 t, b, n;
    SPC_DEV explicit Onb(f3 normal) {
        n = normal;
        if (fabsf(n.x) > fabsf(n.z)) b = mk3(-n.y, n.x, 0.0f);
        else b = mk3(0.0f, -n.z, n.y);
        b = normalize(b);
        t = cross(b, n);
    }
    SPC_DEV f3 to_world(f3 p) const { return p.x * t + p.y * b + p.z * n; }
};
SPC_DEV f3 cosine_sample_hemisphere(float u1, float u2) {
    const float r = sqrtf(u1);
    const float phi = 2.0f * kPi * u2;
    float s, c;
    sincosf(phi, &s, &c);
    f3 p;
    p.x = r * c; p.y = r * s;
    p.z = sqrtf(fmaxf(0.0f, 1.0f - p.x * p.x - p.y * p.y));
    return p;
}
SPC_DEV float schlick(float u) { float m = clampf(1.0f - u, 0.0f, 1.0f); float m2 = m * m; return m2 * m2 * m; }
SPC_DEV float gtr1(float NdH, float a) {
    if (a >= 1.0f) return kInvPi;
    float a2 = a * a;
    float t = 1.0f + (a2 - 1.0f) * NdH * NdH;
    return (a2 - 1.0f) / (kPi * logf(a2) * t);
}
SPC_DEV float gtr2(float NdH, float a) {
    float a2 = a * a;
    float t = 1.0f + (a2 - 1.0f) * NdH * NdH;
    return a2 / (kPi * t * t);
}
SPC_DEV float smith_ggx(float NdV, float alphaG) {
    float a = alphaG * alphaG, b = NdV * NdV;
    return 1.0f / (NdV + sqrtf(a + b - a * b));
}
SPC_DEV f3 bsdf_eval(const Pbr& m, f3 N, f3 V, f3 L) {
    const float NdL = dot(N, L), NdV = dot(N, V);
    if (NdL <= 0.0f || NdV <= 0.0f) return mk3(0.0f);
    const f3 H = normalize(L + V);
    const float NdH = dot(N, H), LdH = dot(L, H);
    const f3 Cd = m.base;
    const float lum = 0.3f * Cd.x + 0.6f * Cd.y + 0.1f * Cd.z;
    const f3 Ctint = lum > 0.0f ? Cd / lum : mk3(1.0f);
    const f3 Cspec0 = lerp3(m.specular * 0.08f * lerp3(mk3(1.0f), Ctint, m.specularTint), Cd, m.metallic);
    const float FL = schlick(NdL), FV = schlick(NdV);
    const float Fd90 = 0.5f + 2.0f * LdH * LdH * m.roughness;
    const float Fd = lerpf(1.0f, Fd90, FL) * lerpf(1.0f, Fd90, FV);
    const float Fss90 = LdH * LdH * m.roughness;
    const float Fss = lerpf(1.0f, Fss90, FL) * lerpf(1.0f, Fss90, FV);
    const float ss = 1.25f * (Fss * (1.0f / (NdL + NdV) - 0.5f) + 0.5f);
    const float a = fmaxf(0.001f, m.roughness);
    const float Ds = gtr2(NdH, a);
    const float FH = schlick(LdH);
    const f3 Fs = lerp3(Cspec0, mk3(1.0f), FH);
    const float rg = (m.roughness * 0.5f + 0.5f) * (m.roughness * 0.5f + 0.5f);
    const float Gs = smith_ggx(NdL, rg) * smith_ggx(NdV, rg);
    f3 out = ((kInvPi * lerpf(Fd, ss, m.subsurface)) * Cd) * (1.0f - m.metallic) + Gs * Fs * Ds;
    if (m.sheen != 0.0f) {
        const f3 Csheen = lerp3(mk3(1.0f), Ctint, m.sheenTint);
        out = ((kInvPi * lerpf(Fd, ss, m.subsurface)) * Cd + FH * m.sheen * Csheen) * (1.0f - m.metallic) + Gs * Fs * Ds;
    }
    if (m.clearcoat != 0.0f) {
        const float Dr = gtr1(NdH, lerpf(0.1f, 0.001f, m.clearcoatGloss));
        const float Fr = lerpf(0.04f, 1.0f, FH);
        const float Gr = smith_ggx(NdL, 0.25f) * smith_ggx(NdV, 0.25f);
        out = out + mk3(0.25f * m.clearcoat * Gr * Fr * Dr);
    }
    return out;
}
template <bool ENV = true>
SPC_DEV f3 brdf_div(const Pbr& m, f3 f, f3 n, f3 dir) {
// ... 34 lines not shown
```

### spcbpt-optix7_amd/csrc/dev_sampling.h

```cpp
#pragma once
#include "device_lib.h"

namespace spc {

template <bool COUNT>
SPC_DEV int tree_label(const float* tree, f3 position, f3 normal, f3 dir, Counts<COUNT>& cn) {
    if (!tree) return 0;
    int node = 0;
    while (true) {
        const float4 q = ldq(tree, (size_t)node);
        cn.add(C_TREE);
        const uint32_t meta = __float_as_uint(q.w);
        if (meta & TREE_LEAF_BIT) return (int)(meta & ~TREE_LEAF_BIT);
        const uint32_t type = (meta >> 29) & 3u;
        const f3 p = type == 0 ? position : (type == 1 ? normal : dir);
        node = (int)(meta & 0x1fffffffu) + (p.x > q.x ? 1 : 0) + (p.y > q.y ? 2 : 0) + (p.z > q.z ? 4 : 0);
    }
}

template <bool COUNT, bool NODIR = false>
SPC_DEV void tree_label2(const float* treeA, f3 posA, f3 nA, f3 dirA, bool needA, const float* treeB, f3 posB, f3 nB, f3 dirB, bool needB,
                         int& labelA, int& labelB, Counts<COUNT>& cn) {
    int nodeA = 0, nodeB = 0;
    bool goA = needA && treeA != nullptr, goB = needB && treeB != nullptr;
    labelA = 0; labelB = 0;
    float4 a = make_float4(0.0f, 0.0f, 0.0f, 0.0f), b = a;
    while (goA || goB) {
        if (goA) { a = ldq(treeA, (size_t)nodeA); cn.add(C_TREE); }
        if (goB) { b = ldq(treeB, (size_t)nodeB); cn.add(C_TREE); }
#define SPC_TREE_STEP__(q, pos, nrm, dir, node, label, go)                                                              \
        {                                                                                                             \
            const uint32_t meta = __float_as_uint(q.w);                                                               \
            const bool leaf = (meta & TREE_LEAF_BIT) != 0u;                                                           \
            const uint32_t type = (meta >> 29) & 3u;                                                                  \
            const f3 p = NODIR ? mk3(type != 0u ? nrm.x : pos.x, type != 0u ? nrm.y : pos.y, type != 0u ? nrm.z : pos.z)  \
                               : (type == 0u ? pos : (type == 1u ? nrm : dir));                                       \
            const int next = (int)(meta & 0x1fffffffu) + (p.x > q.x ? 1 : 0) + (p.y > q.y ? 2 : 0) + (p.z > q.z ? 4 : 0);   \
            label = (go && leaf) ? (int)(meta & ~TREE_LEAF_BIT) : label;                                              \
            node = (go && !leaf) ? next : node;                                                                       \
            go = go && !leaf;                                                                                         \
        }
        SPC_TREE_STEP__(a, posA, nA, dirA, nodeA, labelA, goA)
        SPC_TREE_STEP__(b, posB, nB, dirB, nodeB, labelB, goB)
#undef SPC_TREE_STEP__
    }
}


template <bool COUNT>
SPC_DEV float gamma_ss(const KParams& p, int e, int l, Counts<COUNT>& cn) {
    if (p.gamma_q) { cn.add(C_GQ, 1); return p.gamma_q[(size_t)e * SPCBPT_NUM_SUBSPACE + l]; }
    const float* row = p.cmf_gamma + (size_t)e * SPCBPT_NUM_SUBSPACE;
    const float g = l == 0 ? row[0] : row[l] - row[l - 1];
    cn.add(C_GQ, l == 0 ? 2 : 3);
    return g / p.Q[l];
}

template <bool COUNT>
SPC_DEV int binary_sample(const float* cmf, int size, uint32_t& seed, float& pmf, Counts<COUNT>& cn) {
    const float index = rnd(seed);
    int mid = size / 2 - 1, l = 0, r = size;
    while (r - l > 1) {
        cn.add(C_CMF);
        if (index < cmf[mid]) r = mid + 1;
        else l = mid + 1;
        mid = (l + r) / 2 - 1;
    }
    pmf = l == 0 ? cmf[l] : cmf[l] - cmf[l - 1];
    return l;
}

SPC_DEV int uniform_sample_index(int vertex_count, uint32_t& seed, float& pmf) {
    pmf = (float)(1.0 / (double)vertex_count);
    return min((int)(rnd(seed) * (float)vertex_count), vertex_count - 1);
}
SPC_DEV int uniform_sample(const int32_t* jump, int vertex_count, uint32_t& seed, float& pmf) {
    return jump[uniform_sample_index(vertex_count, seed, pmf)];
}

static constexpr int GUIDE_WINDOW = 8;
struct GuideScan { int cnt; float lo, hi; };
template <bool RANGE = true>
SPC_DEV void guide_window(float4 q0, float4 q1, int pos, int first, int end, float u, GuideScan& s) {
    const float v[8] = {q0.x, q0.y, q0.z, q0.w, q1.x, q1.y, q1.z, q1.w};
#pragma unroll
    for (int i = 0; i < GUIDE_WINDOW; i++) {
        const bool in = !RANGE || ((i >= 3 || pos + i >= first) && pos + i < end);
        const bool le = in && v[i] <= u, gt = in && !(v[i] <= u);
        s.cnt += le ? 1 : 0;
        s.lo = fmaxf(s.lo, le ? v[i] : -INFINITY);
        s.hi = fminf(s.hi, gt ? v[i] : INFINITY);
    }
}
SPC_DEV int sample_first_stage_guided(const float* cmf_gamma2, const uint16_t* guide1, int eye_subspace, float u, int& l, float& pmf) {
    const float* fine = cmf_gamma2 + (size_t)eye_subspace * CMF2_ROW + CMF2_COARSE + CMF2_MID;
    const int g = guide1[(size_t)eye_subspace * CMF_GUIDE1 + (int)(u * (float)CMF_GUIDE1)];
    const int c0 = max(g - 1, 0);
    int pos = c0 & ~3, windows = 0;
    GuideScan s = {pos, -INFINITY, INFINITY};
    do {
        const float4 q0 = *reinterpret_cast<const float4*>(fine + pos), q1 = *reinterpret_cast<const float4*>(fine + pos + 4);
        guide_window<false>(q0, q1, pos, c0, CMF2_FINE, u, s);
        pos += GUIDE_WINDOW; windows++;
    } while (!(s.hi < INFINITY) && pos < CMF2_FINE);
    l = s.cnt;
    pmf = l == 0 ? s.hi : s.hi - s.lo;
// ... 23 lines not shown
```

### spcbpt-optix7_amd/csrc/eye_walk.h

```cpp
#pragma once
#include "device_lib.h"

namespace spc {

struct WalkState {
    f3 origin, dir;
    f3 next_flux;
    float next_single_pdf;
    uint32_t seed;
    bool done;
};

template <bool COUNT, bool CACHE = false, bool ENV = true>
SPC_DEV void eye_surface_hit(const KParams& p, const Geom& g, float t_hit, f3 ray_dir, bool last_is_origin, const EyeVertex& last,
                             WalkState& w, EyeVertex& mid, Counts<COUNT>& cn, bool stop_dead_paths = false) {
    const DeviceScene& S = p.scene;
    Pbr pbr = load_pbr(S, g.mat);
    color_tex_sample(S, g, pbr, cn);
    f3 N = g.N;
    if (dot(N, ray_dir) > 0.f) N = -N;
    const f3 inv_dir = -ray_dir;
    const f3 new_dir = bsdf_sample(pbr, N, inv_dir, w.seed);
    const float pdf = bsdf_pdf(pbr, N, inv_dir, new_dir);
    if (!(pdf > 0.0f)) w.done = true;

    mid.c.pos = g.P;
    mid.c.n = N;
    const float pdf_G = fabsf(dot(N, ray_dir) * dot(last.c.n, ray_dir)) / (t_hit * t_hit);
    mid.flux = last_is_origin ? last.flux * pdf_G : w.next_flux * last.flux * pdf_G;
    mid.c.lastPos = last.c.pos;
    mid.c.color = pbr.base;
    mid.c.lnp = fabsf(dot(last.c.n, ray_dir));
    mid.c.lld = false;
    mid.c.mat = g.mat;
    int light_label;
    mid.lsub = 0;
    if (CACHE) {
        tree_label2<COUNT, true>(p.eye_tree, g.P, N, inv_dir, true, p.light_tree, g.P, N, inv_dir, last.depth + 1 != 1, mid.sub, mid.lsub, cn);
        light_label = last.lsub;
    } else {
        tree_label2(p.eye_tree, g.P, N, inv_dir, true, p.light_tree, last.c.pos, last.c.n, normalize(g.P - last.c.pos),
                    last.depth + 1 != 1 && last.depth != 1, mid.sub, light_label, cn);
    }
    mid.lastZone = last.sub;
    mid.depth = last.depth + 1;
    mid.singlePdf = w.next_single_pdf * pdf_G / fabsf(dot(last.c.n, ray_dir));
    mid.pdf = last.pdf * mid.singlePdf;
    if (mid.depth == 1) {
        mid.R3 = mk3(0.0f);
    } else {
        const Pbr mat_last = load_pbr_colored(S, last.c.mat, last.c.color);
        const f3 in_dir = normalize(mid.c.pos - last.c.pos);
        const float LL_pdf = rmis_last_pdf(mat_last, last.c, in_dir);
        const float wgt = rmis_weight_eye_l(p, last.depth, last.lastZone, light_label, cn);
        const f3 fm = rmis_flux_multiplier<ENV>(mat_last, last.c, in_dir, normalize(last.c.lastPos - last.c.pos));
        mid.R3 = (last.R3 * LL_pdf * fm + mk3(wgt)) / last.singlePdf;
    }
    cn.add(C_VERTEX);
    w.next_flux = brdf_div<ENV>(pbr, bsdf_eval(pbr, N, inv_dir, new_dir), N, new_dir);
    if (stop_dead_paths && w.next_flux.x == 0.0f && w.next_flux.y == 0.0f && w.next_flux.z == 0.0f) w.done = true;
    w.next_single_pdf = pdf;
    w.origin = g.P;
    w.dir = new_dir;
    const float r = rnd(w.seed);
    const float rr = rr_of(mid.c.color);
    if (r > rr) w.done = true;
    else w.next_single_pdf *= rr;
}

template <bool COUNT, bool CACHE = false, bool ENV = true>
SPC_DEV f3 eye_emitter_hit(const KParams& p, const Geom& g, float t_hit, f3 ray_dir, bool last_is_origin, const EyeVertex& last,
                           const WalkState& w, Counts<COUNT>& cn) {
    const DeviceScene& S = p.scene;
    const int light_id = load_pbr(S, g.mat).light_id;
    const DLight& L = S.lights[light_id];
    const bool mesh = ENV && L.type == 2;
    const f3 ln = mesh ? g.N : ld3(L.normal);
    if (dot(ray_dir, ln) > 0) return mk3(0.0f);
    const LightSampleD ls = mesh ? mesh_light_at_hit(S, L, g) : light_reverse_sample(S, L, g.u, g.v);
    const float pdf_G = fabsf(dot(ln, ray_dir) * dot(last.c.n, ray_dir)) / (t_hit * t_hit);
    const f3 flux = last_is_origin ? last.flux * pdf_G * ls.emission : w.next_flux * last.flux * pdf_G * ls.emission;
    const float singlePdf = w.next_single_pdf * pdf_G / fabsf(dot(last.c.n, ray_dir));
    const float pdf = last.pdf * singlePdf;
    float rmis_pointer = 1.0f;
    if (last.depth + 1 != 1) {
        const f3 lpos = g.P;
        const f3 connect_dir = normalize(last.c.pos - lpos);
        const f3 lflux = ls.emission / ls.pdf;
        const Pbr mat_e = load_pbr_colored(S, last.c.mat, last.c.color);
        const f3 LB = normalize(last.c.lastPos - last.c.pos);
        const float LL_pdf_A = rmis_last_pdf(mat_e, last.c, -connect_dir);
        const f3 fm0 = rmis_flux_multiplier<ENV>(mat_e, last.c, -connect_dir, LB);
        const float wA = CACHE ? rmis_weight_eye_l(p, last.depth, last.lastZone, last.lsub, cn) : rmis_weight_eye(p, last.c, last.depth, last.lastZone, lpos, cn);
        const f3 D_A_0 = last.R3 * LL_pdf_A * fm0 + mk3(wA);
        const float pdf_A = rmis_pdf_from_light(lpos, ln, last.c.pos, last.c.n);
        const float D_A = sum3(D_A_0 * pdf_A * kPi * lflux / last.singlePdf);
        const float weight = sum3(gamma_ss(p, last.sub, ls.subspace, cn) * lflux * (float)SPCBPT_CONNECTION_N);
        const float D_B = 1.0f;
        const float pdf_B = rmis_get_pdf(mat_e, last.c, lpos, ln, LB);
        const float lh = D_B / ((weight + D_A) / pdf_B * ls.pdf + D_B);
        rmis_pointer = 1.0f / lh;
    }
    const f3 ans = flux / pdf / rmis_pointer;
    return is_invalid(ans) ? mk3(0.0f) : ans;
}

template <bool COUNT, bool CACHE = false, bool ENV = true>
SPC_DEV f3 eye_sky_miss(const KParams& p, f3 ray_dir, bool last_is_origin, const EyeVertex& last, const WalkState& w, Counts<COUNT>& cn,
                        float* w_out = nullptr, int* label_out = nullptr) {
    const DeviceScene& S = p.scene;
    const f3 Le = env_color(S.env, ray_dir);
    const float light_pdf = env_pdf(S.env, ray_dir) / (float)S.n_lights;
    const int label = env_label(S.env, ray_dir);
    const float pdf_G = fabsf(dot(last.c.n, ray_dir));
    const f3 flux = last_is_origin ? last.flux * pdf_G * Le : w.next_flux * last.flux * pdf_G * Le;
    const float singlePdf = w.next_single_pdf * pdf_G / fabsf(dot(last.c.n, ray_dir));
    const float pdf = last.pdf * singlePdf;
    float rmis_pointer = 1.0f;
    if (last.depth + 1 != 1) {
        const f3 lflux = Le / light_pdf;
        const Pbr mat_e = load_pbr_colored(S, last.c.mat, last.c.color);
// ... 44 lines not shown
```

### spcbpt-optix7_amd/csrc/kernels.h

```cpp
#pragma once
#include <hip/hip_runtime.h>

#include <algorithm>

#include "layout.h"

namespace spc {

int render_thread_count(const KParams& p);
int spcbpt_block_threads();
void launch_spcbpt(const KParams& p, int variant, int max_blocks, hipStream_t s);
int spcbpt_blocks_per_cu(int variant, bool batch, bool general, bool sky);
bool eye_sees_sky(const KParams& p);
int render_tile_count(const KParams& p);
void launch_pt(const KParams& p, bool count, hipStream_t s);
void launch_film_merge(const KParams& p, hipStream_t s);
void launch_light_trace(const KParams& p, int variant, int max_blocks, hipStream_t s);
struct CompactBatch { LightVertex* lvc[kMaxBatchFrames]; int* counts[kMaxBatchFrames]; };
void launch_lvc_compact_batch(const LightVertex* scratch, const int* core_counts, const int* core_offsets, const int* path_counts, int core_count,
                              int core_padding, int n, const CompactBatch& dst, int capacity, uint32_t* overflow, hipStream_t s);
int light_trace_blocks(const KParams& p, int max_blocks);
void launch_lvc_compact(const LightVertex* scratch, const int* core_counts, const int* core_offsets, int core_count, int core_padding,
                        LightVertex* lvc, uint32_t* keys, uint32_t* vals, float* weights, int* sampler_counts, int capacity, uint32_t* overflow,
                        hipStream_t s);
void launch_fill_keys(const LightVertex* lvc, int n, uint32_t* keys, uint32_t* vals, float* weights, int* sampler_counts, hipStream_t s);
void launch_fill_keys_devcount(const LightVertex* lvc, int bound, uint32_t* keys, uint32_t* vals, float* weights, const int* sampler_counts, hipStream_t s);
void launch_gather_compact(const LightVertex* gathered, const int* counts_all, int world, int cap, int lvc_capacity, const CompactBatch& dst, int nf,
                           int* overflow, hipStream_t s);
void launch_pack_shards(const CompactBatch& src, int nf, int cap, LightVertex* send, int* send_counts, hipStream_t s);
struct MergeBatch { const float* result[kMaxBatchFrames]; uint32_t subframe[kMaxBatchFrames]; };
void launch_film_merge_batch(const KParams& p, const MergeBatch& m, int frames, hipStream_t s);
void launch_pack_bands(float* accum, int width, int height, int rank, int world, float* packed, bool unpack_all, hipStream_t s);
size_t sampler_build_hist_ints();
struct SamplerBuildBatch {
    const LightVertex* lvc[kMaxBatchFrames]; const int* n_dev[kMaxBatchFrames]; int* path_count[kMaxBatchFrames];
    DSubspace* sub[kMaxBatchFrames]; uint32_t* jump[kMaxBatchFrames]; float* cmfs[kMaxBatchFrames];
    LightVertex* lvc_sorted[kMaxBatchFrames];
    uint32_t* guide[kMaxBatchFrames];
    int n_host[kMaxBatchFrames];
    uint32_t* keys; float* weights; int* hist; double* wsorted; size_t item_stride;
};
void launch_sampler_build_batch(const SamplerBuildBatch& b, int frames, hipStream_t s);
void launch_sampler_build(const LightVertex* lvc, int n_host, const int* n_dev, uint32_t* keys, float* weights, int* hist, int* path_count, DSubspace* sub,
                          uint32_t* jump, double* wsorted, float* cmfs, LightVertex* lvc_sorted, uint32_t* guide, hipStream_t s);
void launch_sampler_guide(const DSubspace* sub, const float* cmfs, uint32_t* guide, hipStream_t s);
void launch_lvc_sorted_copy(const LightVertex* lvc, const uint32_t* jump, const int* sampler_counts, LightVertex* lvc_sorted, int capacity, hipStream_t s);
void launch_subspace_ranges(const uint32_t* sorted_keys, const int* sampler_counts, DSubspace* sub, int capacity, hipStream_t s);
void launch_gather_weights(const float* weights, const uint32_t* sorted_vals, const int* sampler_counts, double* out, int capacity, hipStream_t s);
void launch_cmf(const double* prefix, const uint32_t* sorted_keys, const int* sampler_counts, DSubspace* sub, float* cmfs, int capacity, hipStream_t s);
int spcbpt_batch_blocks(const KParams& p, int max_blocks);
void launch_spcbpt_batch(const KParams& p, int max_blocks, hipStream_t s);
void launch_trace_closest(const KParams& p, const float* rays, int n, float* t, int* tri, float* uv, hipStream_t s);
void launch_pretrace(const KParams& p, uint32_t iteration, int num_core, int padding, spcbpt_pretrace_path* paths,
                     spcbpt_pretrace_node* nodes, hipStream_t s);
void launch_trace_any(const KParams& p, const float* rays, int n, int* vis, hipStream_t s);

void launch_spcbpt_no_rmis(const KParams& p, hipStream_t s);

void launch_repack_nodes_quad(const float* nodes, float* out, int n_nodes, hipStream_t s);
int trace_bench_blocks_per_cu(int mode, bool any);
void launch_trace_bench(const KParams& p, int mode, bool any, bool stats, const float* nodes_q, const float* rays, int n, uint32_t* counter, float* t, int* tri,
                        float* uv, int* vis, unsigned long long* stat_out, int blocks, hipStream_t s);

void launch_unit(const KParams& p, int op, const uint32_t* in, int in_words, uint32_t* out, int out_words, int n, const float* aux, hipStream_t s);

#ifndef SPC_STACK_LDS
#define SPC_STACK_LDS 16
#endif
static const int kStackLds = SPC_STACK_LDS;

}
```

### spcbpt-optix7_amd/csrc/kernels_light.hip

```cpp
#include <hip/hip_runtime.h>

#include "device_lib.h"
#include "eye_walk.h"
#include "kernel_config.h"
#include "kernels.h"

namespace spc {

template <bool COUNT, bool CACHE>
__global__ __launch_bounds__(BLOCK, SPC_WAVES) void k_light_trace(const KParams p) {
    __shared__ uint32_t s_stack[BLOCK * STACK_LDS];
    if (SPC_PRIO_LIGHT) __builtin_amdgcn_s_setprio(SPC_PRIO_LIGHT);
    const DeviceScene& S = p.scene;
    const uint32_t lane = threadIdx.x & 63;
    Counts<COUNT> cn;
    cn.clear();
    TravStack<BLOCK, STACK_LDS> st;
    st.init(s_stack, p.spill, p.spill_entries, (size_t)blockIdx.x * BLOCK + threadIdx.x, p.diag);
    int paths_started = 0;
    bool has_core = false, exhausted = false;
    int local_core = 0, nverts = 0, npaths = 0, origins = 0;
    uint32_t seed = 0, pseed = 0;
    LightVertex* slots = nullptr;
    const bool batched = p.n_lframes > 0;
// ... 32 lines not shown
                pool_base = t;
                pool_left = min(64, (int)(queue_len - t));
            }
            const int n_idle = __popcll(idle);
            const int take = n_idle < pool_left ? n_idle : pool_left;
            const int my_rank = __popcll(idle & ((1ull << lane) - 1ull));
            if (!has_core && my_rank < take) {
                local_core = (int)pool_base + my_rank;
                has_core = true;
                uint32_t launch_frame = p.launch_frame;
                LightVertex* scratch = p.lvc_scratch;
                if (batched) {
                    fk = local_core / p.core_count;
                    local_core -= fk * p.core_count;
                    launch_frame += (uint32_t)fk;
                    scratch += (size_t)fk * p.core_count * p.core_padding;
                }
                const int core = p.core_begin + local_core;
                seed = tea4((uint32_t)core, launch_frame);
                pseed = p.lt_decorrelate ? tea4((uint32_t)core ^ 0x80000000u, launch_frame) : seed;
                slots = scratch + (size_t)local_core * p.core_padding;
                nverts = 0; npaths = 0; origins = 0;
                in_path = false;
            }
            pool_base += (uint32_t)take;
            pool_left -= take;
            idle = __ballot(!has_core);
        }
        if (!__any(has_core)) break;
        if (has_core && !in_path) {
            const int lid = pick_light(S, seed);
            const DLight& L = S.lights[lid];
            LightSampleD ls;
            float dir_pdf;
            uint32_t origin_flags = 0u;
            if (L.type == 1) {
                ls = env_light_sample(S, seed, dir_pdf);
                dir = ls.normal;
                origin_flags = SPCBPT_LV_DIRECTION;
            } else {
                ls = area_light_sample(S, L, seed);
                const float d1 = rnd(seed), d2 = rnd(seed);
                const Onb onb(ls.normal);
                dir = onb.to_world(cosine_sample_hemisphere(d1, d2));
                dir_pdf = fabsf(dot(dir, ls.normal)) * kInvPi;
            }
            origin = ls.position;
            path_id = (uint32_t)(p.core_begin + local_core) * (uint32_t)p.m_per_core + (uint32_t)npaths;
            cn.add(C_LIGHT);
            LightVertex v;
            v.position[0] = ls.position.x; v.position[1] = ls.position.y; v.position[2] = ls.position.z; v.pdf = ls.pdf;
            v.normal[0] = ls.normal.x; v.normal[1] = ls.normal.y; v.normal[2] = ls.normal.z; v.single_pdf = ls.pdf;
            v.flux[0] = ls.emission.x; v.flux[1] = ls.emission.y; v.flux[2] = ls.emission.z; v.rmis_pointer = 1.0f;
            v.color[0] = v.color[1] = v.color[2] = 0.0f; v.last_lum = 0.0f;
            v.last_position[0] = v.last_position[1] = v.last_position[2] = 0.0f; v.last_normal_projection = 0.0f;
            v.material_id = (int16_t)L.id; v.subspace_id = (int16_t)ls.subspace; v.depth = 0; v.last_zone_id = 0;
            v.path_id = path_id; v.pad = origin_flags;
            store(v);
            origins++;
            last = v;
            next_flux = mk3(0.0f);
            next_single_pdf = dir_pdf;
            depth = 0;
            in_path = nverts < p.core_padding;
            if (!in_path) { core_done(); has_core = false; }
        }
        const bool tracing = has_core && in_path;
        HitRec h;
        h.tri = -1;
        if (tracing) {
            cn.add(C_CLOSEST);
            traverse<false, COUNT>(S, st, origin, dir, kEps, 1e16f, h, cn);
        }
        if (tracing) {
            bool done = false, full = false;
            if (h.tri < 0) { done = true; }
            else {
                const Geom g = local_geometry(S, h);
                if (g.emitter) { done = true; }
                else {
                    Pbr pbr = load_pbr(S, g.mat);
                    color_tex_sample(S, g, pbr, cn);
                    f3 N = g.N;
                    if (dot(N, dir) > 0.f) N = -N;
                    const f3 inv_dir = -dir;
                    const f3 new_dir = bsdf_sample(pbr, N, inv_dir, pseed);
                    const float pdf = bsdf_pdf(pbr, N, inv_dir, new_dir);
                    if (!(pdf > 0.0f)) done = true;
                    const f3 last_n = ld3(last.normal), last_flux = ld3(last.flux);
                    const bool last_dir = (last.pad & SPCBPT_LV_DIRECTION) != 0u;
                    const float pdf_G = last_dir ? fabsf(dot(N, dir) * dot(last_n, dir)) : fabsf(dot(N, dir) * dot(last_n, dir)) / (h.t * h.t);
                    const f3 flux = last.depth == 0 ? last_flux * pdf_G : next_flux * last_flux * pdf_G;
                    LightVertex m;
                    m.position[0] = g.P.x; m.position[1] = g.P.y; m.position[2] = g.P.z;
                    m.normal[0] = N.x; m.normal[1] = N.y; m.normal[2] = N.z;
                    m.flux[0] = flux.x; m.flux[1] = flux.y; m.flux[2] = flux.z;
                    m.color[0] = pbr.base.x; m.color[1] = pbr.base.y; m.color[2] = pbr.base.z;
                    m.last_position[0] = last.position[0]; m.last_position[1] = last.position[1]; m.last_position[2] = last.position[2];
                    if (last_dir) { const f3 lp = g.P - dir; m.last_position[0] = lp.x; m.last_position[1] = lp.y; m.last_position[2] = lp.z; }
                    m.last_normal_projection = fabsf(dot(last_n, dir));
                    m.material_id = (int16_t)g.mat;
                    int new_label, eye_label;
                    const f3 last_pos = ld3(last.position);
                    uint32_t own_eye_label = 0u;
                    if (CACHE) {
                        int own;
                        tree_label2<COUNT, true>(p.light_tree, g.P, N, inv_dir, true, p.eye_tree, g.P, N, inv_dir, true, new_label, own, cn);
                        own_eye_label = (uint32_t)own + 1u;
                        eye_label = (int)(last.pad & 0xffffu) - 1;
                    } else {
                        tree_label2(p.light_tree, g.P, N, inv_dir, true, p.eye_tree, last_pos, last_n, normalize(g.P - last_pos), last.depth != 0,
                                    new_label, eye_label, cn);
                    }
                    m.subspace_id = (int16_t)new_label;
                    m.last_zone_id = last.subspace_id;
                    m.depth = (int16_t)(last.depth + 1);
                    m.single_pdf = next_single_pdf * pdf_G / fabsf(dot(last_n, dir));
                    m.pdf = last.pdf * m.single_pdf;
                    m.last_lum = sum3(last_flux / last.pdf);
                    m.path_id = path_id; m.pad = own_eye_label | (last_dir ? SPCBPT_LV_LAST_DIRECTION : 0u);
                    if (last.depth == 0) {
                        m.rmis_pointer = last.rmis_pointer / last.single_pdf;
                    } else {
                        const VCore lc = core_of(last);
                        const Pbr mat_last = load_pbr_colored(S, lc.mat, lc.color);
                        const f3 in_dir = normalize(g.P - lc.pos);
                        const float LL_pdf = rmis_last_pdf(mat_last, lc, in_dir);
                        const float wgt = rmis_weight_light_l(p, last.last_zone_id, last.last_lum, eye_label, cn);
                        m.rmis_pointer = (last.rmis_pointer * LL_pdf + wgt) / last.single_pdf;
                    }
                    cn.add(C_VERTEX);
                    next_flux = brdf_div(pbr, bsdf_eval(pbr, N, inv_dir, new_dir), N, new_dir);
                    next_single_pdf = pdf;
                    origin = g.P;
                    dir = new_dir;
                    const float r = rnd(pseed);
                    const float rr = rr_of(pbr.base);
                    if (r > rr) done = true;
                    else next_single_pdf *= rr;
                    store(m);
                    last = m;
                    if (!(nverts < p.core_padding)) full = true;
                }
            }
            bool path_over = full;
            if (!full) {
                if (done || depth > 50) path_over = true;
                else depth += 1;
            }
            if (path_over) {
                in_path = false;
                bool core_over = full;
                if (!full) {
                    npaths++;
                    if (npaths >= p.m_per_core || !(nverts < p.core_padding)) core_over = true;
                }
                if (core_over) { core_done(); has_core = false; }
            }
        }
    }
    for (int o = 32; o > 0; o >>= 1) paths_started += __shfl_down(paths_started, o, 64);
    if (lane == 0 && paths_started) atomicAdd(p.path_counter, paths_started);
    cn.flush(p.counters);
}

__global__ void k_lvc_compact(const LightVertex* __restrict__ scratch, const int* __restrict__ core_counts,
                              const int* __restrict__ core_offsets, int core_count, int core_padding, LightVertex* __restrict__ lvc,
                              uint32_t* __restrict__ keys, uint32_t* __restrict__ vals, float* __restrict__ weights,
                              int* __restrict__ sampler_counts, int capacity, uint32_t* __restrict__ overflow) {
    const long long t = (long long)blockIdx.x * blockDim.x + threadIdx.x;
    if (t == 0 && core_offsets[core_count] > capacity) { sampler_counts[0] = capacity; *overflow = 1u; }
    if (t < (long long)core_count * core_padding) {
        const int core = (int)(t / core_padding), slot = (int)(t % core_padding);
        if (slot < core_counts[core] && core_offsets[core] + slot < capacity) {
            const int dst_i = core_offsets[core] + slot;
            const float4* src = reinterpret_cast<const float4*>(scratch + t);
            float4* dst = reinterpret_cast<float4*>(lvc + dst_i);
            float4 q[6];
#pragma unroll
            for (int k = 0; k < 6; k++) q[k] = src[k];
#pragma unroll
            for (int k = 0; k < 6; k++) dst[k] = q[k];
            const LightVertex& v = *reinterpret_cast<const LightVertex*>(q);
            float w = (v.flux[0] + v.flux[1] + v.flux[2]) / v.pdf;
            if (isinf(w) || isnan(w)) w = 0.0f;
            keys[dst_i] = (uint32_t)v.subspace_id;
            vals[dst_i] = (uint32_t)dst_i;
            weights[dst_i] = w;
        }
    }
// ... 190 lines not shown
```

### spcbpt-optix7_amd/csrc/kernels_sampler.hip

```cpp
#include <hip/hip_runtime.h>

#include "device_lib.h"
#include "eye_walk.h"
#include "kernel_config.h"
#include "kernels.h"

namespace spc {

__global__ void k_subspace_ranges(const uint32_t* __restrict__ sorted_keys, const int* __restrict__ sampler_counts, DSubspace* __restrict__ sub) {
    const int n = sampler_counts[0];
    const int i = blockIdx.x * blockDim.x + threadIdx.x;
    if (i >= n) return;
    const uint32_t k = sorted_keys[i];
    if (i == 0 || sorted_keys[i - 1] != k) sub[k].jump_bias = i;
    if (i == n - 1 || sorted_keys[i + 1] != k) sub[k].size = i + 1;
}
__global__ void k_finish_ranges(DSubspace* __restrict__ sub) {
    __shared__ int ends[1024];
    const int s = threadIdx.x;
    const int end = s < SPCBPT_NUM_SUBSPACE ? sub[s].size : 0;
    ends[s] = end;
    __syncthreads();
    for (int off = 1; off < 1024; off <<= 1) {
        const int v = s >= off ? ends[s - off] : 0;
// ... 163 lines not shown
    if (sz <= 0) return;
    double acc = 0.0;
    for (int j = t; j < sz; j += 256) acc += wsorted[b + j];
    sh[t] = acc;
    __syncthreads();
    for (int off = 128; off > 0; off >>= 1) { if (t < off) sh[t] += sh[t + off]; __syncthreads(); }
    const double total = sh[0];
    __syncthreads();
    double carry = 0.0;
    for (int j0 = 0; j0 < sz; j0 += 256) {
        const int j = j0 + t;
        const double w = j < sz ? wsorted[b + j] : 0.0;
        sh[t] = w;
        __syncthreads();
        for (int off = 1; off < 256; off <<= 1) {
            const double v = t >= off ? sh[t - off] : 0.0;
            __syncthreads();
            sh[t] += v;
            __syncthreads();
        }
        if (j < sz) {
            float c = total > 0.0 ? (float)((carry + sh[t]) / total) : (float)(j + 1) / (float)sz;
            if (j == sz - 1) c = 1.0f;
            cmfs[b + j] = c;
        }
        carry += sh[255];
        __syncthreads();
    }
    if (t == 0) sub[k].sum_pmf = (float)total;
    if (B.guide[blockIdx.y]) build_guide(cmfs + b, sz, B.guide[blockIdx.y] + b, t, 256);
}
__global__ __launch_bounds__(256) void k_sb_guide(const DSubspace* __restrict__ sub, const float* cmfs, uint32_t* __restrict__ guide) {
    const int b = sub[blockIdx.x].jump_bias, sz = sub[blockIdx.x].size;
    if (sz > 0) build_guide(cmfs + b, sz, guide + b, threadIdx.x, 256);
}
void launch_sampler_guide(const DSubspace* sub, const float* cmfs, uint32_t* guide, hipStream_t s) {
    if (guide) hipLaunchKernelGGL(k_sb_guide, dim3(SPCBPT_NUM_SUBSPACE), dim3(256), 0, s, sub, cmfs, guide);
}
size_t sampler_build_hist_ints() { return (size_t)(SB_BLOCKS + 1) * 1024; }
void launch_sampler_build_batch(const SamplerBuildBatch& b, int frames, hipStream_t s) {
    if (frames <= 0) return;
    hipLaunchKernelGGL(k_sb_hist, dim3(SB_BLOCKS, frames), dim3(64), 0, s, b);
    hipLaunchKernelGGL(k_sb_scan, dim3(1, frames), dim3(1024), 0, s, b);
    hipLaunchKernelGGL(k_sb_scatter, dim3(SB_BLOCKS, frames), dim3(64), 0, s, b);
    hipLaunchKernelGGL(k_sb_cmf, dim3(SPCBPT_NUM_SUBSPACE, frames), dim3(256), 0, s, b);
    hipLaunchKernelGGL(k_sb_copy, dim3(256, frames), dim3(256), 0, s, b);
}
__global__ __launch_bounds__(256) void k_lvc_sorted_copy(const LightVertex* __restrict__ lvc, const uint32_t* __restrict__ jump, const int* __restrict__ counts,
                                                        LightVertex* __restrict__ out, int capacity) {
    const int n = min(counts[0], capacity);
    const float4* src = reinterpret_cast<const float4*>(lvc);
    float4* dst = reinterpret_cast<float4*>(out);
    for (int i = blockIdx.x * 256 + threadIdx.x; i < n; i += gridDim.x * 256) {
        const size_t from = jump[i];
#pragma unroll
        for (int q = 0; q < 6; q++) dst[(size_t)i * 6 + q] = src[from * 6 + q];
    }
}
void launch_lvc_sorted_copy(const LightVertex* lvc, const uint32_t* jump, const int* sampler_counts, LightVertex* lvc_sorted, int capacity, hipStream_t s) {
    if (capacity <= 0 || !lvc_sorted) return;
    hipLaunchKernelGGL(k_lvc_sorted_copy, dim3(512), dim3(256), 0, s, lvc, jump, sampler_counts, lvc_sorted, capacity);
}
void launch_sampler_build(const LightVertex* lvc, int n_host, const int* n_dev, uint32_t* keys, float* weights, int* hist, int* path_count, DSubspace* sub,
                          uint32_t* jump, double* wsorted, float* cmfs, LightVertex* lvc_sorted, uint32_t* guide, hipStream_t s) {
    SamplerBuildBatch b = {};
    b.guide[0] = guide;
    b.lvc[0] = lvc; b.n_host[0] = n_host; b.n_dev[0] = n_dev; b.path_count[0] = path_count; b.sub[0] = sub; b.jump[0] = jump; b.cmfs[0] = cmfs;
    b.lvc_sorted[0] = lvc_sorted;
    b.keys = keys; b.weights = weights; b.hist = hist; b.wsorted = wsorted; b.item_stride = 0;
    launch_sampler_build_batch(b, 1, s);
}

void launch_subspace_ranges(const uint32_t* sorted_keys, const int* sampler_counts, DSubspace* sub, int capacity, hipStream_t s) {
    hipLaunchKernelGGL(k_subspace_ranges, dim3((capacity + 255) / 256), dim3(256), 0, s, sorted_keys, sampler_counts, sub);
    hipLaunchKernelGGL(k_finish_ranges, dim3(1), dim3(1024), 0, s, sub);
}
void launch_gather_weights(const float* weights, const uint32_t* sorted_vals, const int* sampler_counts, double* out, int capacity, hipStream_t s) {
    hipLaunchKernelGGL(k_gather_weights, dim3((capacity + 255) / 256), dim3(256), 0, s, weights, sorted_vals, sampler_counts, out);
}
void launch_cmf(const double* prefix, const uint32_t* sorted_keys, const int* sampler_counts, DSubspace* sub, float* cmfs, int capacity, hipStream_t s) {
    hipLaunchKernelGGL(k_cmf, dim3((capacity + 255) / 256), dim3(256), 0, s, prefix, sorted_keys, sampler_counts, sub, cmfs);
}

}
```

Baseline: 644.7 Mpaths/s.

## Precompute per-triangle subspace tree start nodes to shorten tree descent

Adds a per-triangle table, stored just before the triangle records, that holds the deepest eye-tree and light-tree node each triangle falls wholly inside, for both normal orientations. A kernel builds the table when the subspace trees are installed. Eye and light walks then begin tree_label2 from these nodes instead of the root. This cuts the tree traversal loads per vertex, at the cost of one extra 8-byte load per hit, some extra memory, and a conservative double-precision margin test to keep the labels unchanged.

```diff
diff --git a/include/spcbpt.h b/include/spcbpt.h
--- a/include/spcbpt.h
+++ b/include/spcbpt.h
@@ -312,6 +312,8 @@
 int spcbpt_build_sampler_batch(spcbpt_ctx* ctx, int n_builds);
 int spcbpt_debug_batch_scratch(spcbpt_ctx* ctx, int64_t* bytes, int* frames, int* fallbacks);
 int spcbpt_debug_read_sampling_tables(spcbpt_ctx* ctx, uint32_t* guide2, int capacity2, uint16_t* guide1, float* gamma_q);
+int spcbpt_debug_read_tri_starts(spcbpt_ctx* ctx, uint32_t* starts, float* records, int capacity, float* eye_tree, float* light_tree,
+                                 int tree_capacity, int32_t* n_triangles, int32_t* n_eye_nodes, int32_t* n_light_nodes);
 
 int spcbpt_set_light_ahead(spcbpt_ctx* ctx, int on);
 int spcbpt_get_pipeline_state(spcbpt_ctx* ctx, int* light_ahead, int* pending_passes, int* sampler_intact, int* deferred_outstanding);
diff --git a/spcbpt-optix7_amd/api.py b/spcbpt-optix7_amd/api.py
--- a/spcbpt-optix7_amd/api.py
+++ b/spcbpt-optix7_amd/api.py
@@ -703,6 +703,7 @@
         "spcbpt_read_film": [vp, vp, vp],
         "spcbpt_debug_batch_scratch": [vp, C.POINTER(C.c_int64), C.POINTER(i32), C.POINTER(i32)],
         "spcbpt_debug_read_sampling_tables": [vp, vp, i32, vp, vp],
+        "spcbpt_debug_read_tri_starts": [vp, vp, vp, i32, vp, vp, i32, C.POINTER(i32), C.POINTER(i32), C.POINTER(i32)],
         "spcbpt_lvc_import_wait": [vp],
         "spcbpt_kernel_time": [vp, C.c_char_p, C.POINTER(C.c_double), C.POINTER(i32)],
         "spcbpt_reset_kernel_time": [vp],
@@ -794,7 +795,7 @@
     "spcbpt_lvc_export", "spcbpt_lvc_import", "spcbpt_lvc_set_capacity", "spcbpt_lvc_get_capacity", "spcbpt_set_environment", "spcbpt_get_environment", "spcbpt_set_environment_mode", "spcbpt_get_environment_mode", "spcbpt_hdr_load", "spcbpt_lvc_read", "spcbpt_sampler_read", "spcbpt_read_accum",
     "spcbpt_read_frame", "spcbpt_accum_device_ptr", "spcbpt_clear_accum", "spcbpt_get_counters",
     "spcbpt_reset_counters", "spcbpt_debug_phase_clocks", "spcbpt_debug_spill_arm", "spcbpt_debug_spill_count", "spcbpt_set_connection_sampler", "spcbpt_debug_unit", "spcbpt_debug_trace_bench",
-    "spcbpt_build_source_hash", "spcbpt_build_arithmetic", "spcbpt_abi_struct_sizes", "spcbpt_lvc_export_on", "spcbpt_lvc_import_gathered", "spcbpt_lvc_export_batch_on", "spcbpt_lvc_import_gathered_batch", "spcbpt_film_pack_bands", "spcbpt_film_unpack_bands", "spcbpt_image_size", "spcbpt_get_light_trace", "spcbpt_enable_counters", "spcbpt_stream", "spcbpt_sync", "spcbpt_sync_light", "spcbpt_launch_deferred", "spcbpt_merge_deferred", "spcbpt_sync_film", "spcbpt_set_light_ahead", "spcbpt_get_pipeline_state", "spcbpt_reuse_sampler", "spcbpt_read_film", "spcbpt_debug_batch_scratch", "spcbpt_debug_read_sampling_tables", "spcbpt_lvc_import_wait", "spcbpt_kernel_time",
+    "spcbpt_build_source_hash", "spcbpt_build_arithmetic", "spcbpt_abi_struct_sizes", "spcbpt_lvc_export_on", "spcbpt_lvc_import_gathered", "spcbpt_lvc_export_batch_on", "spcbpt_lvc_import_gathered_batch", "spcbpt_film_pack_bands", "spcbpt_film_unpack_bands", "spcbpt_image_size", "spcbpt_get_light_trace", "spcbpt_enable_counters", "spcbpt_stream", "spcbpt_sync", "spcbpt_sync_light", "spcbpt_launch_deferred", "spcbpt_merge_deferred", "spcbpt_sync_film", "spcbpt_set_light_ahead", "spcbpt_get_pipeline_state", "spcbpt_reuse_sampler", "spcbpt_read_film", "spcbpt_debug_batch_scratch", "spcbpt_debug_read_sampling_tables", "spcbpt_debug_read_tri_starts", "spcbpt_lvc_import_wait", "spcbpt_kernel_time",
     "spcbpt_reset_kernel_time", "spcbpt_enable_kernel_timing", "spcbpt_trace_closest", "spcbpt_trace_any", "spcbpt_camera_splat",
     "spcbpt_launch_features", "spcbpt_read_features", "spcbpt_denoise", "spcbpt_denoise_params_struct_size", "spcbpt_read_denoised", "spcbpt_denoise_host",
     "spcbpt_set_film_moments", "spcbpt_get_film_moments", "spcbpt_read_film_moments", "spcbpt_film_moments_update_host", "spcbpt_film_error", "spcbpt_film_error_struct_size", "spcbpt_film_error_host", "spcbpt_denoise_variance", "spcbpt_denoise_variance_host",
@@ -1087,6 +1088,18 @@
         self._chk(self.lib.spcbpt_debug_read_sampling_tables(self.h, g2.ctypes.data if vertex_count > 0 else None, len(g2), g1.ctypes.data, gq.ctypes.data),
                   "debug_read_sampling_tables")
         return g2[:vertex_count], g1, gq
+
+    def tri_starts(self):
+        n, ne, nl = C.c_int32(), C.c_int32(), C.c_int32()
+        self._chk(self.lib.spcbpt_debug_read_tri_starts(self.h, None, None, 0, None, None, 0, C.byref(n), C.byref(ne), C.byref(nl)), "debug_read_tri_starts")
+        starts = np.zeros((n.value, 4), dtype=np.uint32)
+        rec = np.zeros((n.value, 16), dtype=np.float32)
+        cap = max(ne.value, nl.value, 1)
+        et, lt = np.zeros((cap, 4), dtype=np.float32), np.zeros((cap, 4), dtype=np.float32)
+        have = ne.value > 0
+        self._chk(self.lib.spcbpt_debug_read_tri_starts(self.h, starts.ctypes.data, rec.ctypes.data, n.value, et.ctypes.data if have else None,
+                                                        lt.ctypes.data if have else None, cap, C.byref(n), C.byref(ne), C.byref(nl)), "debug_read_tri_starts")
+        return starts, rec, et[:ne.value].copy(), lt[:nl.value].copy()
 
     def lvc_read(self, capacity=None):
         if capacity is None:
diff --git a/spcbpt-optix7_amd/csrc/capi.hip b/spcbpt-optix7_amd/csrc/capi.hip
--- a/spcbpt-optix7_amd/csrc/capi.hip
+++ b/spcbpt-optix7_amd/csrc/capi.hip
@@ -200,7 +200,10 @@
     c->n_lights = (int)lights.size(); c->n_mats = (int)mats.size();
 
     CREATE_TRY(c->d_nodes.reserve(bvh.nodes.size() + bvh.pairs.size()));
-    CREATE_TRY(c->d_tris.reserve(bvh.tris.size()));
+    const size_t start_floats = (size_t)mesh.n_triangles * 4;
+    CREATE_TRY(c->d_tris.reserve(start_floats + bvh.tris.size()));
+    CREATE_TRY(hipMemset(c->d_tris, 0, start_floats * 4));
+    if (const char* e = getenv("SPCBPT_TRI_STARTS")) c->tri_starts = atoi(e) != 0;
     if (getenv("SPCBPT_NO_TRI_PAIRS")) {
         for (size_t i = 0; i < bvh.pairs.size() / 16; i++) { uint32_t fl; memcpy(&fl, &bvh.pairs[i * 16 + 15], 4); fl &= 0x80000000u; memcpy(&bvh.pairs[i * 16 + 15], &fl, 4); }
         bvh.n_paired = 0;
@@ -210,7 +213,7 @@
     CREATE_TRY(c->d_tri_orig.reserve(bvh.tri_orig.size()));
     CREATE_TRY(c->d_mats.reserve(mats.size()));
     CREATE_TRY(hipMemcpy(c->d_nodes, bvh.nodes.data(), bvh.nodes.size() * 4, hipMemcpyHostToDevice));
-    CREATE_TRY(hipMemcpy(c->d_tris, bvh.tris.data(), bvh.tris.size() * 4, hipMemcpyHostToDevice));
+    CREATE_TRY(hipMemcpy(c->d_tris + start_floats, bvh.tris.data(), bvh.tris.size() * 4, hipMemcpyHostToDevice));
     CREATE_TRY(hipMemcpy(c->d_tri_orig, bvh.tri_orig.data(), bvh.tri_orig.size() * 4, hipMemcpyHostToDevice));
     CREATE_TRY(hipMemcpy(c->d_mats, mats.data(), mats.size() * sizeof(DMaterial), hipMemcpyHostToDevice));
     c->h_lights = lights;
@@ -249,7 +252,7 @@
     CREATE_TRY(hipMemset(c->d_counters, 0, C_COUNT * sizeof(unsigned long long)));
     memset(&c->kp, 0, sizeof(c->kp));
     if (c->upload_lights()) { g_create_error = c->error; delete c; return SPCBPT_ERR_HIP; }
-    c->kp.scene.nodes = c->d_nodes; c->kp.scene.tris = c->d_tris; c->kp.scene.tri_base = c->n_nodes; c->kp.scene.tri_orig = c->d_tri_orig; c->kp.scene.mats = c->d_mats;
+    c->kp.scene.nodes = c->d_nodes; c->kp.scene.tris = c->d_tris + start_floats; c->kp.scene.tri_base = c->n_nodes; c->kp.scene.tri_orig = c->d_tri_orig; c->kp.scene.mats = c->d_mats;
     c->kp.scene.lights = c->d_lights; c->kp.scene.tex = c->d_tex; c->kp.scene.n_lights = c->n_lights; c->kp.scene.n_mats = c->n_mats;
     CREATE_TRY(c->d_nodes_q.reserve((size_t)c->n_nodes * 16));
     launch_repack_nodes_quad(c->d_nodes, c->d_nodes_q, c->n_nodes, c->stream);
diff --git a/spcbpt-optix7_amd/csrc/capi_debug.hip b/spcbpt-optix7_amd/csrc/capi_debug.hip
--- a/spcbpt-optix7_amd/csrc/capi_debug.hip
+++ b/spcbpt-optix7_amd/csrc/capi_debug.hip
@@ -95,6 +95,29 @@
     if ((guide1 || gamma_q) && !c->d_guide1) { c->error = "no subspace tuple installed"; return SPCBPT_ERR_STATE; }
     if (guide1) HIP_TRY(c, hipMemcpy(guide1, c->d_guide1, (size_t)SPCBPT_NUM_SUBSPACE * CMF_GUIDE1 * sizeof(uint16_t), hipMemcpyDeviceToHost));
     if (gamma_q) HIP_TRY(c, hipMemcpy(gamma_q, c->d_gamma_q, (size_t)SPCBPT_NUM_SUBSPACE * SPCBPT_NUM_SUBSPACE * sizeof(float), hipMemcpyDeviceToHost));
+    return SPCBPT_OK;
+}
+int spcbpt_debug_read_tri_starts(spcbpt_ctx* c, uint32_t* starts, float* records, int capacity, float* eye_tree, float* light_tree, int tree_capacity,
+                                 int32_t* n_triangles, int32_t* n_eye_nodes, int32_t* n_light_nodes) {
+    CTX_CHECK(c);
+    if (c->sync_all()) return SPCBPT_ERR_HIP;
+    if (n_triangles) *n_triangles = c->n_triangles;
+    if (n_eye_nodes) *n_eye_nodes = c->have_subspace ? c->n_eye_tree_slots : 0;
+    if (n_light_nodes) *n_light_nodes = c->have_subspace ? c->n_light_tree_slots : 0;
+    if ((starts || records) && capacity < c->n_triangles) { c->error = "debug_read_tri_starts: buffer too small"; return SPCBPT_ERR_CAPACITY; }
+    const size_t n = (size_t)c->n_triangles;
+    if (starts) {
+        std::vector<uint32_t> h(n * 4);
+        HIP_TRY(c, hipMemcpy(h.data(), c->d_tris, n * 16, hipMemcpyDeviceToHost));
+        for (size_t t = 0; t < n; t++) memcpy(starts + 4 * t, &h[(n - 1 - t) * 4], 16);
+    }
+    if (records) HIP_TRY(c, hipMemcpy(records, c->kp.scene.tris, n * 64, hipMemcpyDeviceToHost));
+    if (eye_tree || light_tree) {
+        if (!c->have_subspace) { c->error = "no subspace tuple installed"; return SPCBPT_ERR_STATE; }
+        if (tree_capacity < std::max(c->n_eye_tree_slots, c->n_light_tree_slots)) { c->error = "debug_read_tri_starts: tree buffer too small"; return SPCBPT_ERR_CAPACITY; }
+        if (eye_tree) HIP_TRY(c, hipMemcpy(eye_tree, c->d_eye_tree, (size_t)c->n_eye_tree_slots * 16, hipMemcpyDeviceToHost));
+        if (light_tree) HIP_TRY(c, hipMemcpy(light_tree, c->d_light_tree, (size_t)c->n_light_tree_slots * 16, hipMemcpyDeviceToHost));
+    }
     return SPCBPT_OK;
 }
 int spcbpt_accum_device_ptr(spcbpt_ctx* c, void** p) {
diff --git a/spcbpt-optix7_amd/csrc/context.h b/spcbpt-optix7_amd/csrc/context.h
--- a/spcbpt-optix7_amd/csrc/context.h
+++ b/spcbpt-optix7_amd/csrc/context.h
@@ -148,6 +148,8 @@
     DevBuf<float> d_nodes_q;
     DevBuf<float> d_nodes_q2;
     DevBuf<float> d_tris;
+    bool tri_starts = true;
+    int build_tri_starts();
     int n_paired = 0;
     DevBuf<int32_t> d_tri_orig;
     DevBuf<DMaterial> d_mats;
@@ -168,6 +170,7 @@
     bool have_camera = false;
     float* d_eye_tree = nullptr;
     float* d_light_tree = nullptr;
+    int n_eye_tree_slots = 0, n_light_tree_slots = 0;
     DevBuf<float> d_Q;
     DevBuf<float> d_gamma;
     DevBuf<float> d_gamma2;
@@ -215,7 +218,7 @@
     int ensure_spill(size_t threads, bool render = false);
     int ensure_temp(size_t bytes);
     int ensure_lvc_capacity(size_t n);
-    int upload_tree(const spcbpt_tree_node* t, int n, float*& d_tree, std::vector<spcbpt_tree_node>& host_copy);
+    int upload_tree(const spcbpt_tree_node* t, int n, float*& d_tree, std::vector<spcbpt_tree_node>& host_copy, int& n_slots);
     int install_subspace(const spcbpt_tree_node* et, int ne, const spcbpt_tree_node* lt, int nl, const float* q, const float* g);
     int install_minimal_tuple();
     int set_light_trace(const spcbpt_light_trace_params& p);
diff --git a/spcbpt-optix7_amd/csrc/ctx_state.hip b/spcbpt-optix7_amd/csrc/ctx_state.hip
--- a/spcbpt-optix7_amd/csrc/ctx_state.hip
+++ b/spcbpt-optix7_amd/csrc/ctx_state.hip
@@ -75,7 +75,7 @@
     return 0;
 }
 
-int Context::upload_tree(const spcbpt_tree_node* t, int n, float*& d_tree, std::vector<spcbpt_tree_node>& host_copy) {
+int Context::upload_tree(const spcbpt_tree_node* t, int n, float*& d_tree, std::vector<spcbpt_tree_node>& host_copy, int& n_slots) {
     for (int i = 0; i < n; i++) {
         if (t[i].leaf) {
             if (t[i].label < 0 || t[i].label >= SPCBPT_NUM_SUBSPACE) { error = "tree label out of range"; return SPCBPT_ERR_INVALID_ARG; }
@@ -109,19 +109,33 @@
     HIP_TRY(this, dev_alloc(&d_tree, packed.size()));
     HIP_TRY(this, hipMemcpyAsync(d_tree, packed.data(), packed.size() * sizeof(float), hipMemcpyHostToDevice, stream));
     HIP_TRY(this, hipStreamSynchronize(stream));
+    n_slots = (int)src.size();
+    return 0;
+}
+
+int Context::build_tri_starts() {
+    if (!tri_starts || n_triangles == 0) return 0;
+    float* table = d_tris;
+    if (tree_has_direction) HIP_TRY(this, hipMemsetAsync(table, 0, (size_t)n_triangles * 16, stream));
+    else {
+        launch_tri_starts(kp.scene.tris, n_triangles, d_eye_tree, d_light_tree, stream);
+        HIP_TRY(this, hipGetLastError());
+    }
     return 0;
 }
 
 int Context::install_subspace(const spcbpt_tree_node* et, int ne, const spcbpt_tree_node* lt, int nl, const float* q, const float* g) {
     if (!et || !lt || !q || !g || ne < 1 || nl < 1) { error = "set_subspace: all four of eye_tree, light_tree, q, cmf_gamma are required"; return SPCBPT_ERR_INVALID_ARG; }
     if (sync_all()) return SPCBPT_ERR_HIP;
-    int rc = upload_tree(et, ne, d_eye_tree, h_eye_tree);
+    int rc = upload_tree(et, ne, d_eye_tree, h_eye_tree, n_eye_tree_slots);
     if (rc) return rc;
-    rc = upload_tree(lt, nl, d_light_tree, h_light_tree);
+    rc = upload_tree(lt, nl, d_light_tree, h_light_tree, n_light_tree_slots);
     if (rc) return rc;
     tree_has_direction = false;
     for (int i = 0; i < ne; i++) if (!et[i].leaf && et[i].type == 2) tree_has_direction = true;
     for (int i = 0; i < nl; i++) if (!lt[i].leaf && lt[i].type == 2) tree_has_direction = true;
+    rc = build_tri_starts();
+    if (rc) return rc;
     h_Q.assign(q, q + SPCBPT_NUM_SUBSPACE);
     h_gamma.assign(g, g + (size_t)SPCBPT_NUM_SUBSPACE * SPCBPT_NUM_SUBSPACE);
     HIP_TRY(this, d_Q.reserve(SPCBPT_NUM_SUBSPACE));
diff --git a/spcbpt-optix7_amd/csrc/dev_bsdf.h b/spcbpt-optix7_amd/csrc/dev_bsdf.h
--- a/spcbpt-optix7_amd/csrc/dev_bsdf.h
+++ b/spcbpt-optix7_amd/csrc/dev_bsdf.h
@@ -42,7 +42,7 @@
     r.z = w00 * (((t00 >> 16) & 255u) * s) + w10 * (((t10 >> 16) & 255u) * s) + w01 * (((t01 >> 16) & 255u) * s) + w11 * (((t11 >> 16) & 255u) * s);
     return r;
 }
-struct Geom { f3 P, N; float u, v; int mat; bool emitter; };
+struct Geom { f3 P, N; float u, v; int mat; bool emitter; int tri; };
 SPC_DEV Geom local_geometry(const DeviceScene& S, const HitRec& h) {
     const size_t base = (size_t)h.tri * 4;
     const float4 a = ldq(S.tris, base), b = ldq(S.tris, base + 1), c = ldq(S.tris, base + 2), d = ldq(S.tris, base + 3);
@@ -56,7 +56,11 @@
     const uint32_t meta = __float_as_uint(d.w);
     g.mat = (int)(meta & 0x7fffffffu);
     g.emitter = (meta & 0x80000000u) != 0;
+    g.tri = h.tri;
     return g;
+}
+SPC_DEV uint2 tri_start(const DeviceScene& S, int tri, bool flipped) {
+    return *reinterpret_cast<const uint2*>(reinterpret_cast<const uint32_t*>(S.tris) - ((size_t)tri + 1) * 4 + (flipped ? 2 : 0));
 }
 template <bool COUNT>
 SPC_DEV void color_tex_sample(const DeviceScene& S, const Geom& g, Pbr& m, Counts<COUNT>& cn) {
diff --git a/spcbpt-optix7_amd/csrc/dev_sampling.h b/spcbpt-optix7_amd/csrc/dev_sampling.h
--- a/spcbpt-optix7_amd/csrc/dev_sampling.h
+++ b/spcbpt-optix7_amd/csrc/dev_sampling.h
@@ -20,8 +20,8 @@
 
 template <bool COUNT, bool NODIR = false>
 SPC_DEV void tree_label2(const float* treeA, f3 posA, f3 nA, f3 dirA, bool needA, const float* treeB, f3 posB, f3 nB, f3 dirB, bool needB,
-                         int& labelA, int& labelB, Counts<COUNT>& cn) {
-    int nodeA = 0, nodeB = 0;
+                         int& labelA, int& labelB, Counts<COUNT>& cn, int startA = 0, int startB = 0) {
+    int nodeA = startA, nodeB = startB;
     bool goA = needA && treeA != nullptr, goB = needB && treeB != nullptr;
     labelA = 0; labelB = 0;
     float4 a = make_float4(0.0f, 0.0f, 0.0f, 0.0f), b = a;
diff --git a/spcbpt-optix7_amd/csrc/eye_walk.h b/spcbpt-optix7_amd/csrc/eye_walk.h
--- a/spcbpt-optix7_amd/csrc/eye_walk.h
+++ b/spcbpt-optix7_amd/csrc/eye_walk.h
@@ -18,7 +18,10 @@
     Pbr pbr = load_pbr(S, g.mat);
     color_tex_sample(S, g, pbr, cn);
     f3 N = g.N;
-    if (dot(N, ray_dir) > 0.f) N = -N;
+    const bool flipped = dot(N, ray_dir) > 0.f;
+    if (flipped) N = -N;
+    uint2 start = make_uint2(0u, 0u);
+    if (CACHE && !COUNT) start = tri_start(S, g.tri, flipped);
     const f3 inv_dir = -ray_dir;
     const f3 new_dir = bsdf_sample(pbr, N, inv_dir, w.seed);
     const float pdf = bsdf_pdf(pbr, N, inv_dir, new_dir);
@@ -36,7 +39,8 @@
     int light_label;
     mid.lsub = 0;
     if (CACHE) {
-        tree_label2<COUNT, true>(p.eye_tree, g.P, N, inv_dir, true, p.light_tree, g.P, N, inv_dir, last.depth + 1 != 1, mid.sub, mid.lsub, cn);
+        tree_label2<COUNT, true>(p.eye_tree, g.P, N, inv_dir, true, p.light_tree, g.P, N, inv_dir, last.depth + 1 != 1, mid.sub, mid.lsub, cn,
+                                 (int)start.x, (int)start.y);
         light_label = last.lsub;
     } else {
         tree_label2(p.eye_tree, g.P, N, inv_dir, true, p.light_tree, last.c.pos, last.c.n, normalize(g.P - last.c.pos),
diff --git a/spcbpt-optix7_amd/csrc/kernels.h b/spcbpt-optix7_amd/csrc/kernels.h
--- a/spcbpt-optix7_amd/csrc/kernels.h
+++ b/spcbpt-optix7_amd/csrc/kernels.h
@@ -48,6 +48,7 @@
 void launch_subspace_ranges(const uint32_t* sorted_keys, const int* sampler_counts, DSubspace* sub, int capacity, hipStream_t s);
 void launch_gather_weights(const float* weights, const uint32_t* sorted_vals, const int* sampler_counts, double* out, int capacity, hipStream_t s);
 void launch_cmf(const double* prefix, const uint32_t* sorted_keys, const int* sampler_counts, DSubspace* sub, float* cmfs, int capacity, hipStream_t s);
+void launch_tri_starts(const float* tris, int n_triangles, const float* eye_tree, const float* light_tree, hipStream_t s);
 int spcbpt_batch_blocks(const KParams& p, int max_blocks);
 void launch_spcbpt_batch(const KParams& p, int max_blocks, hipStream_t s);
 void launch_trace_closest(const KParams& p, const float* rays, int n, float* t, int* tri, float* uv, hipStream_t s);
diff --git a/spcbpt-optix7_amd/csrc/kernels_light.hip b/spcbpt-optix7_amd/csrc/kernels_light.hip
--- a/spcbpt-optix7_amd/csrc/kernels_light.hip
+++ b/spcbpt-optix7_amd/csrc/kernels_light.hip
@@ -138,7 +138,10 @@
                     Pbr pbr = load_pbr(S, g.mat);
                     color_tex_sample(S, g, pbr, cn);
                     f3 N = g.N;
-                    if (dot(N, dir) > 0.f) N = -N;
+                    const bool flipped = dot(N, dir) > 0.f;
+                    if (flipped) N = -N;
+                    uint2 start = make_uint2(0u, 0u);
+                    if (CACHE && !COUNT) start = tri_start(S, g.tri, flipped);
                     const f3 inv_dir = -dir;
                     const f3 new_dir = bsdf_sample(pbr, N, inv_dir, pseed);
                     const float pdf = bsdf_pdf(pbr, N, inv_dir, new_dir);
@@ -161,7 +164,7 @@
                     uint32_t own_eye_label = 0u;
                     if (CACHE) {
                         int own;
-                        tree_label2<COUNT, true>(p.light_tree, g.P, N, inv_dir, true, p.eye_tree, g.P, N, inv_dir, true, new_label, own, cn);
+                        tree_label2<COUNT, true>(p.light_tree, g.P, N, inv_dir, true, p.eye_tree, g.P, N, inv_dir, true, new_label, own, cn, (int)start.y, (int)start.x);
                         own_eye_label = (uint32_t)own + 1u;
                         eye_label = (int)(last.pad & 0xffffu) - 1;
                     } else {
diff --git a/spcbpt-optix7_amd/csrc/kernels_sampler.hip b/spcbpt-optix7_amd/csrc/kernels_sampler.hip
--- a/spcbpt-optix7_amd/csrc/kernels_sampler.hip
+++ b/spcbpt-optix7_amd/csrc/kernels_sampler.hip
@@ -269,4 +269,44 @@
     hipLaunchKernelGGL(k_cmf, dim3((capacity + 255) / 256), dim3(256), 0, s, prefix, sorted_keys, sampler_counts, sub, cmfs);
 }
 
-}
+SPC_DEV uint32_t tri_start_node(const float* tree, f3 P0, f3 P1, f3 P2, f3 N) {
+    if (!tree) return 0u;
+    const double lo[3] = {(double)fminf(fminf(P0.x, P1.x), P2.x), (double)fminf(fminf(P0.y, P1.y), P2.y), (double)fminf(fminf(P0.z, P1.z), P2.z)};
+    const double hi[3] = {(double)fmaxf(fmaxf(P0.x, P1.x), P2.x), (double)fmaxf(fmaxf(P0.y, P1.y), P2.y), (double)fmaxf(fmaxf(P0.z, P1.z), P2.z)};
+    uint32_t node = 0u;
+    while (true) {
+        const float4 q = ldq(tree, (size_t)node);
+        const uint32_t meta = __float_as_uint(q.w);
+        if (meta & TREE_LEAF_BIT) return node;
+        const uint32_t type = (meta >> 29) & 3u, first = meta & 0x1fffffffu;
+        if (type == 1u) { node = first + (N.x > q.x ? 1u : 0u) + (N.y > q.y ? 2u : 0u) + (N.z > q.z ? 4u : 0u); continue; }
+        if (type != 0u) return node;
+        const double mid[3] = {(double)q.x, (double)q.y, (double)q.z};
+        uint32_t octant = 0u;
+        for (int k = 0; k < 3; k++) {
+            const double delta = ldexp(fmax(fabs(lo[k]), fabs(hi[k])), -19);
+            if (lo[k] - mid[k] > delta) octant |= 1u << k;
+            else if (!(mid[k] - hi[k] > delta)) return node;
+        }
+        node = first + octant;
+    }
+}
+__global__ __launch_bounds__(256) void k_tri_starts(const float* tris, int n, const float* eye_tree, const float* light_tree) {
+    const int t = blockIdx.x * 256 + threadIdx.x;
+    if (t >= n) return;
+    const size_t base = (size_t)t * 4;
+    const float4 a = ldq(tris, base), b = ldq(tris, base + 1), c = ldq(tris, base + 2);
+    const f3 P0 = mk3(a.x, a.y, a.z), P1 = mk3(b.x, b.y, b.z), P2 = mk3(c.x, c.y, c.z);
+    const f3 N = normalize(cross(P1 - P0, P2 - P0));
+    uint4 e;
+    e.x = tri_start_node(eye_tree, P0, P1, P2, N); e.y = tri_start_node(light_tree, P0, P1, P2, N);
+    e.z = tri_start_node(eye_tree, P0, P1, P2, -N); e.w = tri_start_node(light_tree, P0, P1, P2, -N);
+    uint4* entry = reinterpret_cast<uint4*>(const_cast<float*>(tris)) - ((size_t)t + 1);
+    *entry = e;
+}
+void launch_tri_starts(const float* tris, int n_triangles, const float* eye_tree, const float* light_tree, hipStream_t s) {
+    if (n_triangles <= 0) return;
+    hipLaunchKernelGGL(k_tri_starts, dim3((n_triangles + 255) / 256), dim3(256), 0, s, tris, n_triangles, eye_tree, light_tree);
+}
+
+}
```

Result: no change. 649.2 Mpaths/s (median of 6 runs) (+0.7%).
